# majidsina/rlmd

Measured on NVIDIA B200. Metric: investor-steps/sec (leverage sweep), higher is better.
Workload: dtype 2-bit codes, int32 counts, f64 log-wealth, f32 wealth

## Files before the change

include/rlmd_b200.h:

```cpp
#ifndef RLMD_B200_H
#define RLMD_B200_H

#include <stdint.h>

#ifdef __cplusplus
extern "C" {
#endif

#define B200_OK 0
#define B200_EINVAL (-1)
#define B200_ECUDA (-2)
#define B200_ELIMIT (-3)

#define B200_MAX_PEERS 8

const char* b200_last_error(void);
int b200_version(void);
int b200_device_info(int32_t* sm_count, int32_t* cc_major, int32_t* cc_minor);

enum {
  B200_LEV_DISCRETE = 0,
  B200_LEV_GBM = 1
};
enum {
  B200_SRC_STREAM = 0,
  B200_SRC_PHILOX = 1
};
enum {
  B200_MODE_CHAIN = 1,
  B200_MODE_LOG = 2
};

#define B200_MAX_GRID 64
#define B200_MAX_OUTCOMES 4

typedef struct b200_lev_desc {
  int64_t n_investors;
  int64_t ld_outcomes;
  int64_t investor_offset;
  int64_t ld_out;
  uint64_t seed;
  int32_t horizon;
  int32_t n_grid;
  int32_t n_outcomes;
  int32_t kind;
  int32_t source;
  int32_t mode;
  float value_0;
  float log_mean;
  float sigma;
  int32_t variant;
  uint32_t thresholds[B200_MAX_OUTCOMES];
  int32_t outcome_bits;
  int32_t flags;
} b200_lev_desc;

#define B200_LEV_FLAG_FINAL_ONLY 1
#define B200_LEV_FLAG_STATE_OUT 2
#define B200_LEV_FLAG_BESIDE_SWEEP 4

int b200_lev_sweep(const b200_lev_desc* desc, const void* outcomes,
                   const float* factors_host, float* data_T, double* log_w,
                   int32_t* counts, void* stream);

int b200_lev_chunk(const b200_lev_desc* desc, const void* outcomes,
                   const float* factors_host, int32_t t_begin, int32_t t_end,
                   void* state, float* dump, void* stream);

int b200_lev_draw(const b200_lev_desc* desc, void* out, void* stream);

int b200_lev_from_counts(const b200_lev_desc* desc, const int32_t* counts,
                         const float* factors_host, float* data_T, double* log_w,
                         void* stream);

int b200_lev_pack(const uint8_t* codes, int64_t n_investors, int32_t horizon,
                  int64_t ld_codes, uint8_t* packed, int64_t ld_packed, void* stream);
int b200_lev_pack_bits(const uint8_t* codes, int64_t n_investors, int32_t horizon,
                       int64_t ld_codes, uint8_t* packed, int64_t ld_packed, int32_t bits,
                       void* stream);

typedef struct b200_tally_plan {
  int64_t rows_cap;
  int64_t bins_cap;
  int32_t grid_cap;
  int32_t world;
} b200_tally_plan;

int64_t b200_tally_workspace_bytes(const b200_tally_plan* plan);
int64_t b200_tally_exchange_bytes(const b200_tally_plan* plan);

#define B200_TALLY_INFO_WORDS 8
int b200_tally_reset(const b200_tally_plan* plan, void* workspace, void* stream);

int b200_lev_tally(const b200_lev_desc* desc, const void* outcomes,
                   const b200_tally_plan* plan, void* workspace, int32_t* counts,
                   void* stream);

enum { B200_DT_U8 = 0, B200_DT_I32 = 1, B200_DT_I64 = 2, B200_DT_F32 = 3, B200_DT_F64 = 4 };
int b200_lev_ingest(const void* src, int32_t src_type, int64_t n_investors, int32_t horizon,
                    int64_t ld_src, int32_t n_outcomes, uint8_t* codes, int64_t ld_codes,
                    int32_t* counts, const b200_tally_plan* plan, void* workspace,
                    void* stream);

typedef struct b200_tally_peers {
  void* exchange[B200_MAX_PEERS];
  int32_t world, rank;
  uint32_t epoch;
  uint32_t reserved;
} b200_tally_peers;

int b200_tally_finalize(const b200_tally_plan* plan, void* workspace,
                        const b200_tally_peers* peers, int32_t phase, void* stream);

int b200_tally_stats(const b200_tally_plan* plan, void* workspace, const b200_lev_desc* desc,
                     const float* factors_host, int64_t n_total, int64_t top, double* stats,
                     void* stream);

int64_t b200_rowstats_workspace_bytes(int64_t rows);

int b200_rowstats(const float* values, int64_t rows, int64_t n, int64_t ld,
                  int64_t n_total, int64_t top, void* workspace, double* stats,
                  int32_t phase, void* stream);

int b200_rowstats_exchange(int32_t phase, int64_t out[5]);

enum { B200_ENV_COIN = 0, B200_ENV_DICE = 1, B200_ENV_GBM = 2, B200_ENV_DICE_SH = 3 };
enum { B200_INV_A = 0, B200_INV_B = 1, B200_INV_C = 2, B200_INV_INSURED = 3 };
#define B200_ENV_MAX_GAMBLES 8

typedef struct b200_env_desc {
  int32_t family;
  int32_t investor;
  int32_t n_gambles;
  int32_t stop_abs;
  double max_value, initial_value, min_value;
  double max_abs_action, min_reward, min_return;
  double max_return, min_weight, lev_factor;
  double returns[3];
  double probs[3];
  double sh_returns[3];
  double i_lev_factor, sh_lev_factor;
  double log_mean, vol;
  uint64_t seed;
} b200_env_desc;

int b200_menv_dims(const b200_env_desc* desc, int32_t* state_dim,
                   int32_t* action_dim, int32_t* risk_dim);

int b200_menv_reset(const b200_env_desc* desc, int64_t n_envs, double* wealth,
                    int32_t* time, double* state, const uint8_t* mask, void* stream);

int b200_menv_step(const b200_env_desc* desc, int64_t n_envs, double* wealth,
                   int32_t* time, const double* action, const double* returns_in,
                   uint64_t draw_index, double* next_state, double* reward,
                   uint8_t* done, double* risk, void* stream);

#define B200_REPLAY_MAX_STEPS 64

typedef struct b200_replay_desc {
  int64_t mem_size;
  int32_t state_dim;
  int32_t action_dim;
  float* state_memory;
  float* action_memory;
  float* reward_memory;
  float* next_state_memory;
  uint8_t* terminal_memory;
  int32_t* episode_start;
  int64_t* header;
} b200_replay_desc;

int b200_replay_reset(const b200_replay_desc* desc, void* stream);

int b200_replay_store(const b200_replay_desc* desc, const void* state, const void* action,
                      const void* reward, const void* next_state, const uint8_t* done,
                      int64_t count, int32_t is_f64, int64_t position, double reward_floor,
                      void* stream);

int b200_replay_store_host(const b200_replay_desc* desc, const double* state_host,
                           const double* action_host, double reward,
                           const double* next_state_host, int32_t done, int64_t position,
                           double reward_floor, void* stream);

int b200_replay_sample(const b200_replay_desc* desc, const int64_t* idx, int64_t n_batches,
                       int32_t batch, int64_t filled, int32_t multi_steps,
                       const float* gamma_pow_host, int32_t additive, uint64_t seed,
                       uint64_t draw_index, int64_t* out_idx, float* out_state,
                       float* out_action, float* out_reward, float* out_next_state,
                       uint8_t* out_done, int64_t* out_eff, void* stream);

int b200_replay_sample_counted(const b200_replay_desc* desc, int64_t n_batches, int32_t batch,
                               int32_t multi_steps, const float* gamma_pow_host, int32_t additive,
                               uint64_t seed, int64_t* counter, int64_t* out_idx, float* out_state,
                               float* out_action, float* out_reward, float* out_next_state,
                               uint8_t* out_done, int64_t* out_eff, void* stream);

typedef struct b200_collect_desc {
  b200_env_desc env;
  b200_replay_desc replay;
  int64_t n_envs;
  int64_t lane_len;
  double reward_floor;
} b200_collect_desc;

int b200_collect_reset(const b200_collect_desc* desc, double* wealth, int32_t* time,
                       double* cur_state, int64_t* counter, void* stream);

int b200_collect_step(const b200_collect_desc* desc, double* wealth, int32_t* time,
                      double* cur_state, const double* action, const double* returns_in,
                      int64_t* counter, double* reward, uint8_t* done, double* risk,
                      void* stream);

int b200_collect_sample(const b200_collect_desc* desc, const int64_t* idx, int64_t n_batches,
                        int32_t batch, int32_t multi_steps, const float* gamma_pow_host,
                        int32_t additive, uint64_t seed, int64_t* counter, int64_t* out_idx,
                        float* out_state, float* out_action, float* out_reward,
                        float* out_next_state, uint8_t* out_done, int64_t* out_eff,
                        void* stream);

int b200_menv_rollout(const b200_env_desc* desc, int64_t n_episodes, const double* action,
                      const double* returns_in, uint64_t draw_base, int32_t max_steps,
                      double* reward, int32_t* steps, double* risk, double* last_state,
                      void* stream);

#define B200_MARKET_MAX_ASSETS 128

typedef struct b200_market_desc {
  int32_t investor;
  int32_t n_assets;
  int32_t obs_days;
  int32_t time_length;
  double max_value, initial_value, min_value;
  double max_abs_action, min_reward, min_return;
  double max_return, min_weight, lev_factor;
} b200_market_desc;

int b200_market_dims(const b200_market_desc* desc, int32_t* state_dim, int32_t* action_dim,
                     int32_t* risk_dim);

int b200_market_reset(const b200_market_desc* desc, int64_t n_envs, double* wealth,
                      int32_t* time, const double* assets_in, double* assets, double* state,
                      const uint8_t* mask, void* stream);

int b200_market_step(const b200_market_desc* desc, int64_t n_envs, double* wealth,
                     int32_t* time, const double* assets, const double* action,
                     const double* next_assets, double* next_state, double* reward,
                     uint8_t* done, double* risk, void* stream);

#define B200_PEER_FLAG_ERROR_WORD (B200_MAX_PEERS * 8)
#define B200_PEER_FLAG_WORDS 128
typedef struct b200_peer_set {
  void* workspace[B200_MAX_PEERS];
  uint32_t* flags[B200_MAX_PEERS];
  void* stage[B200_MAX_PEERS];
  int64_t stage_rows;
  int32_t world, rank;
  uint32_t epoch;
  uint32_t reserved;
} b200_peer_set;
int64_t b200_rowstats_stage_bytes(int64_t rows, int32_t world);
int b200_rowstats_p2p(const float* values, int64_t rows, int64_t n, int64_t ld,
                      int64_t n_total, int64_t top, const b200_peer_set* peers,
                      double* stats, void* stream);

int b200_exchange_pack(const void* workspace, int64_t words_per_row, int64_t rows,
                       int64_t int_offset, int64_t int_count, int64_t dbl_offset,
                       int64_t dbl_count, double* staging, void* stream);
int b200_exchange_unpack(void* workspace, int64_t words_per_row, int64_t rows,
                         int64_t int_offset, int64_t int_count, int64_t dbl_offset,
                         int64_t dbl_count, const double* staging, void* stream);

int64_t b200_growth_workspace_bytes(int64_t rows);

int b200_gbm_valid(const double* state, const float* data_T, int64_t n, int64_t ld_T,
                   const float* lev_host, int32_t n_grid, double log_v0, double* out, void* stream);

int b200_gbm_growth_assemble(const double* base_row, const double* valid, const float* lev_host,
                             int32_t n_grid, int32_t horizon, int32_t n_q, const int32_t* pick_pos,
                             const int32_t* pick_neg, double* out, void* stream);
int b200_growth_exchange(int32_t phase, int64_t out[5]);
int b200_growth_summary(const double* log_w, const float* data_T, int64_t rows, int64_t n,
                        int64_t ld, int64_t ld_T, int64_t n_total, double log_v0,
                        int32_t horizon, const double* quantiles_host, int32_t n_q,
                        void* workspace, double* out, int32_t phase, void* stream);

enum { B200_BB_COIN = 0,
       B200_BB_DICE = 1   };
#define B200_BB_MAX_POINTS 128

typedef struct b200_bigbrain_desc {
  int64_t n_investors;
  int64_t ld_outcomes;
  int32_t horizon;
  int32_t n_points;
  int32_t kind;
  int32_t reserved;
  float value_0;
  float lev_factor32;
  double lev_factor64;
  double returns[3];
} b200_bigbrain_desc;

int b200_bigbrain_chunk(const b200_bigbrain_desc* desc, const uint8_t* outcomes,
                        const float* stop_vmin_host, const float* roll_host,
                        const double* lev0_host, int32_t s_begin, int32_t s_end, void* state,
                        float* dump, void* stream);

#ifdef __cplusplus
}
#endif
#endif
```

rlmd_b200/_lib.py:

```python
import ctypes as C
import os

_HERE = os.path.dirname(os.path.abspath(__file__))
LIB_PATH = os.path.join(_HERE, "librlmd_b200.so")

B200_OK, B200_EINVAL, B200_ECUDA, B200_ELIMIT = 0, -1, -2, -3
LEV_DISCRETE, LEV_GBM = 0, 1
SRC_STREAM, SRC_PHILOX = 0, 1
MODE_CHAIN, MODE_LOG = 1, 2
MAX_GRID, MAX_OUTCOMES = 64, 4


class LevDesc(C.Structure):
    _fields_ = [
        ("n_investors", C.c_int64),
        ("ld_outcomes", C.c_int64),
        ("investor_offset", C.c_int64),
        ("ld_out", C.c_int64),
        ("seed", C.c_uint64),
        ("horizon", C.c_int32),
        ("n_grid", C.c_int32),
        ("n_outcomes", C.c_int32),
        ("kind", C.c_int32),
        ("source", C.c_int32),
        ("mode", C.c_int32),
        ("value_0", C.c_float),
        ("log_mean", C.c_float),
        ("sigma", C.c_float),
        ("variant", C.c_int32),
        ("thresholds", C.c_uint32 * MAX_OUTCOMES),
        ("outcome_bits", C.c_int32),
        ("flags", C.c_int32),
    ]


LEV_FLAG_FINAL_ONLY, LEV_FLAG_STATE_OUT, LEV_FLAG_BESIDE_SWEEP = 1, 2, 4
MAX_PEERS = 8


class PeerSet(C.Structure):
    _fields_ = [
        ("workspace", C.c_void_p * MAX_PEERS),
        ("flags", C.c_void_p * MAX_PEERS),
        ("stage", C.c_void_p * MAX_PEERS),
        ("stage_rows", C.c_int64),
        ("world", C.c_int32),
        ("rank", C.c_int32),
        ("epoch", C.c_uint32),
        ("reserved", C.c_uint32),
    ]


class TallyPlan(C.Structure):
    _fields_ = [
        ("rows_cap", C.c_int64),
        ("bins_cap", C.c_int64),
        ("grid_cap", C.c_int32),
        ("world", C.c_int32),
    ]


class TallyPeers(C.Structure):
    _fields_ = [
        ("exchange", C.c_void_p * MAX_PEERS),
        ("world", C.c_int32),
        ("rank", C.c_int32),
        ("epoch", C.c_uint32),
        ("reserved", C.c_uint32),
    ]


DT_U8, DT_I32, DT_I64, DT_F32, DT_F64 = 0, 1, 2, 3, 4
TALLY_INFO_WORDS = 8
TALLY_MAX_HORIZON = (1 << 21) - 1

ENV_COIN, ENV_DICE, ENV_GBM, ENV_DICE_SH = 0, 1, 2, 3
INV_A, INV_B, INV_C, INV_INSURED = 0, 1, 2, 3
ENV_MAX_GAMBLES = 8


class EnvDesc(C.Structure):
    _fields_ = [
        ("family", C.c_int32),
        ("investor", C.c_int32),
        ("n_gambles", C.c_int32),
        ("stop_abs", C.c_int32),
        ("max_value", C.c_double),
        ("initial_value", C.c_double),
        ("min_value", C.c_double),
        ("max_abs_action", C.c_double),
        ("min_reward", C.c_double),
        ("min_return", C.c_double),
        ("max_return", C.c_double),
        ("min_weight", C.c_double),
        ("lev_factor", C.c_double),
        ("returns", C.c_double * 3),
        ("probs", C.c_double * 3),
        ("sh_returns", C.c_double * 3),
        ("i_lev_factor", C.c_double),
        ("sh_lev_factor", C.c_double),
        ("log_mean", C.c_double),
        ("vol", C.c_double),
        ("seed", C.c_uint64),
    ]


REPLAY_MAX_STEPS = 64


class ReplayDesc(C.Structure):
    _fields_ = [
        ("mem_size", C.c_int64),
        ("state_dim", C.c_int32),
        ("action_dim", C.c_int32),
        ("state_memory", C.c_void_p),
        ("action_memory", C.c_void_p),
        ("reward_memory", C.c_void_p),
        ("next_state_memory", C.c_void_p),
        ("terminal_memory", C.c_void_p),
        ("episode_start", C.c_void_p),
        ("header", C.c_void_p),
    ]


class MarketDesc(C.Structure):
    _fields_ = [
        ("investor", C.c_int32),
        ("n_assets", C.c_int32),
        ("obs_days", C.c_int32),
        ("time_length", C.c_int32),
        ("max_value", C.c_double),
        ("initial_value", C.c_double),
        ("min_value", C.c_double),
        ("max_abs_action", C.c_double),
        ("min_reward", C.c_double),
        ("min_return", C.c_double),
        ("max_return", C.c_double),
        ("min_weight", C.c_double),
        ("lev_factor", C.c_double),
    ]


MARKET_MAX_ASSETS = 128


class CollectDesc(C.Structure):
    _fields_ = [
        ("env", EnvDesc),
        ("replay", ReplayDesc),
        ("n_envs", C.c_int64),
        ("lane_len", C.c_int64),
        ("reward_floor", C.c_double),
    ]


BB_COIN, BB_DICE, BB_MAX_POINTS = 0, 1, 128


class BigBrainDesc(C.Structure):
    _fields_ = [
        ("n_investors", C.c_int64),
        ("ld_outcomes", C.c_int64),
        ("horizon", C.c_int32),
        ("n_points", C.c_int32),
        ("kind", C.c_int32),
        ("reserved", C.c_int32),
        ("value_0", C.c_float),
        ("lev_factor32", C.c_float),
        ("lev_factor64", C.c_double),
        ("returns", C.c_double * 3),
    ]


class B200Error(RuntimeError):
    def __init__(self, code, msg):
        super().__init__(f"rlmd_b200 error {code}: {msg}")
        self.code = code


if not os.path.isfile(LIB_PATH):
    raise ImportError(
        f"{LIB_PATH} is missing: build the CUDA library first (make, or __graft_entry__.build()); "
        "rlmd_b200 has no CPU fallback"
    )

lib = C.CDLL(LIB_PATH)

_vp, _i32, _i64 = C.c_void_p, C.c_int32, C.c_int64
_SIGNATURES = {
    "b200_last_error": (C.c_char_p, []),
    "b200_version": (C.c_int, []),
    "b200_device_info": (C.c_int, [C.POINTER(_i32)] * 3),
    "b200_lev_sweep": (C.c_int, [C.POINTER(LevDesc), _vp, C.POINTER(C.c_float), _vp, _vp, _vp, _vp]),
    "b200_lev_draw": (C.c_int, [C.POINTER(LevDesc), _vp, _vp]),
    "b200_lev_from_counts": (C.c_int, [C.POINTER(LevDesc), _vp, C.POINTER(C.c_float), _vp, _vp, _vp]),
    "b200_lev_pack": (C.c_int, [_vp, _i64, _i32, _i64, _vp, _i64, _vp]),
    "b200_lev_pack_bits": (C.c_int, [_vp, _i64, _i32, _i64, _vp, _i64, _i32, _vp]),
    "b200_lev_chunk": (C.c_int, [C.POINTER(LevDesc), _vp, C.POINTER(C.c_float), _i32, _i32, _vp, _vp, _vp]),
    "b200_menv_dims": (C.c_int, [C.POINTER(EnvDesc)] + [C.POINTER(_i32)] * 3),
    "b200_menv_reset": (C.c_int, [C.POINTER(EnvDesc), _i64, _vp, _vp, _vp, _vp, _vp]),
    "b200_menv_step": (C.c_int, [C.POINTER(EnvDesc), _i64, _vp, _vp, _vp, _vp, C.c_uint64, _vp, _vp, _vp, _vp, _vp]),
    "b200_replay_reset": (C.c_int, [C.POINTER(ReplayDesc), _vp]),
    "b200_replay_store": (C.c_int, [C.POINTER(ReplayDesc), _vp, _vp, _vp, _vp, _vp, _i64, _i32, _i64, C.c_double, _vp]),
    "b200_replay_store_host": (C.c_int, [C.POINTER(ReplayDesc), C.POINTER(C.c_double), C.POINTER(C.c_double),
                                         C.c_double, C.POINTER(C.c_double), _i32, _i64, C.c_double, _vp]),
    "b200_replay_sample": (C.c_int, [C.POINTER(ReplayDesc), _vp, _i64, _i32, _i64, _i32, C.POINTER(C.c_float), _i32,
                                     C.c_uint64, C.c_uint64, _vp, _vp, _vp, _vp, _vp, _vp, _vp, _vp]),
    "b200_replay_sample_counted": (C.c_int, [C.POINTER(ReplayDesc), _i64, _i32, _i32, C.POINTER(C.c_float), _i32,
                                             C.c_uint64, _vp, _vp, _vp, _vp, _vp, _vp, _vp, _vp, _vp]),
    "b200_exchange_pack": (C.c_int, [_vp, _i64, _i64, _i64, _i64, _i64, _i64, _vp, _vp]),
    "b200_exchange_unpack": (C.c_int, [_vp, _i64, _i64, _i64, _i64, _i64, _i64, _vp, _vp]),
    "b200_market_dims": (C.c_int, [C.POINTER(MarketDesc)] + [C.POINTER(_i32)] * 3),
    "b200_market_reset": (C.c_int, [C.POINTER(MarketDesc), _i64, _vp, _vp, _vp, _vp, _vp, _vp, _vp]),
    "b200_market_step": (C.c_int, [C.POINTER(MarketDesc), _i64, _vp, _vp, _vp, _vp, _vp, _vp, _vp, _vp, _vp, _vp]),
    "b200_collect_reset": (C.c_int, [C.POINTER(CollectDesc), _vp, _vp, _vp, _vp, _vp]),
    "b200_collect_step": (C.c_int, [C.POINTER(CollectDesc), _vp, _vp, _vp, _vp, _vp, _vp, _vp, _vp, _vp, _vp]),
    "b200_collect_sample": (C.c_int, [C.POINTER(CollectDesc), _vp, _i64, _i32, _i32, C.POINTER(C.c_float), _i32,
                                      C.c_uint64, _vp, _vp, _vp, _vp, _vp, _vp, _vp, _vp, _vp]),
    "b200_menv_rollout": (C.c_int, [C.POINTER(EnvDesc), _i64, _vp, _vp, C.c_uint64, _i32, _vp, _vp, _vp, _vp, _vp]),
    "b200_bigbrain_chunk": (C.c_int, [C.POINTER(BigBrainDesc), _vp, C.POINTER(C.c_float), C.POINTER(C.c_float),
                                      C.POINTER(C.c_double), _i32, _i32, _vp, _vp, _vp]),
    "b200_growth_workspace_bytes": (_i64, [_i64]),
    "b200_gbm_valid": (C.c_int, [_vp, _vp, _i64, _i64, C.POINTER(C.c_float), _i32, C.c_double, _vp, _vp]),
    "b200_gbm_growth_assemble": (C.c_int, [_vp, _vp, C.POINTER(C.c_float), _i32, _i32, _i32, _vp, _vp, _vp, _vp]),
    "b200_growth_exchange": (C.c_int, [_i32, C.POINTER(_i64)]),
    "b200_growth_summary": (C.c_int, [_vp, _vp, _i64, _i64, _i64, _i64, _i64, C.c_double, _i32, C.POINTER(C.c_double),
                                      _i32, _vp, _vp, _i32, _vp]),
    "b200_tally_workspace_bytes": (_i64, [C.POINTER(TallyPlan)]),
    "b200_tally_exchange_bytes": (_i64, [C.POINTER(TallyPlan)]),
    "b200_tally_reset": (C.c_int, [C.POINTER(TallyPlan), _vp, _vp]),
    "b200_lev_tally": (C.c_int, [C.POINTER(LevDesc), _vp, C.POINTER(TallyPlan), _vp, _vp, _vp]),
    "b200_lev_ingest": (C.c_int, [_vp, _i32, _i64, _i32, _i64, _i32, _vp, _i64, _vp, C.POINTER(TallyPlan), _vp, _vp]),
    "b200_tally_finalize": (C.c_int, [C.POINTER(TallyPlan), _vp, C.POINTER(TallyPeers), _i32, _vp]),
    "b200_tally_stats": (C.c_int, [C.POINTER(TallyPlan), _vp, C.POINTER(LevDesc), C.POINTER(C.c_float), _i64, _i64,
                                   _vp, _vp]),
    "b200_rowstats_workspace_bytes": (_i64, [_i64]),
    "b200_rowstats_stage_bytes": (_i64, [_i64, _i32]),
    "b200_rowstats": (C.c_int, [_vp, _i64, _i64, _i64, _i64, _i64, _vp, _vp, _i32, _vp]),
    "b200_rowstats_exchange": (C.c_int, [_i32, C.POINTER(_i64)]),
    "b200_rowstats_p2p": (C.c_int, [_vp, _i64, _i64, _i64, _i64, _i64, C.POINTER(PeerSet), _vp, _vp]),
}
EXPORTS = _SIGNATURES


def _bind():
    for name, (res, args) in _SIGNATURES.items():
        fn = getattr(lib, name)
        fn.restype = res
        fn.argtypes = args


_bind()


def check(rc: int) -> None:
    if rc != 0:
        raise B200Error(rc, lib.b200_last_error().decode("utf-8", "replace"))


def require_cuda():
    import torch

    if not torch.cuda.is_available():
        raise B200Error(B200_ECUDA, "no CUDA device: rlmd_b200 has no CPU fallback")


def stream_ptr():
    import torch

    raw = getattr(torch._C, "_cuda_getCurrentRawStream", None)
    if raw is not None:
        return C.c_void_p(raw(torch.cuda.current_device()))
    return C.c_void_p(torch.cuda.current_stream().cuda_stream)


def ptr(t):
    return C.c_void_p(0 if t is None else t.data_ptr())
```

rlmd_b200/csrc/tally.cu:

```cuda
#include <cooperative_groups.h>

#include <algorithm>
#include <cstdlib>
#include <cstring>

#include "tally.cuh"

namespace b200 {

struct BinEntry {
  unsigned long long key, count;
};
static_assert(sizeof(BinEntry) == 16, "one 16-byte vector per bin");

constexpr int MERGE_CHUNK = 2048;
constexpr int EX_FLAG_BYTES = 128;

struct LogTable {
  double lm[B200_MAX_OUTCOMES][B200_MAX_GRID];
};

struct TallyLayout {
  long long* header;
  unsigned long long* keysA; uint32_t* countsA; uint64_t capA;
  unsigned long long* ukeys; uint32_t* ucnt;
  float* wbuf; int64_t ldw;
  int64_t list_cap;
  BinEntry* concat; uint32_t* slot_of;
  unsigned long long* keysB; unsigned long long* countsB; uint32_t* posB; uint64_t capB;
  int32_t* blockcnt; int64_t nblk;
  int64_t bytes;
};

static uint64_t pow2_at_least(uint64_t v) {
  uint64_t p = 1;
  while (p < v) p <<= 1;
  return p;
}

static int plan_ok(const b200_tally_plan* p) {
  B200_REQUIRE(p != nullptr, "tally: plan is NULL");
  B200_REQUIRE(p->rows_cap >= 1 && p->rows_cap < ((int64_t)1 << 32), "tally: rows_cap must be in 1..2^32-1");
  B200_REQUIRE(p->bins_cap >= 1 && p->bins_cap < ((int64_t)1 << 31), "tally: bins_cap must be in 1..2^31-1");
  B200_REQUIRE(p->grid_cap >= 1 && p->grid_cap <= B200_MAX_GRID, "tally: grid_cap must be in 1..%d", B200_MAX_GRID);
  B200_REQUIRE(p->world >= 1 && p->world <= B200_MAX_PEERS, "tally: world must be in 1..%d", B200_MAX_PEERS);
  return 0;
}

static TallyLayout layout(const b200_tally_plan& p, void* base) {
  TallyLayout L;
  memset(&L, 0, sizeof(L));
  char* b = (char*)base;
  int64_t off = 0;
  auto take = [&](int64_t bytes) { char* r = b ? b + off : nullptr; off += (bytes + 255) & ~(int64_t)255; return r; };
  L.header = (long long*)take(TH_WORDS * 8);
  L.capA = pow2_at_least((uint64_t)std::max<int64_t>(2048, 2 * std::min(p.rows_cap, p.bins_cap)));
  L.list_cap = (int64_t)(L.capA / 2);
  L.keysA = (unsigned long long*)take((int64_t)L.capA * 8);
  L.countsA = (uint32_t*)take((int64_t)L.capA * 4);
  L.ukeys = (unsigned long long*)take(p.bins_cap * 8);
  L.ucnt = (uint32_t*)take(p.bins_cap * 4);
  L.ldw = (p.bins_cap + 3) & ~(int64_t)3;
  L.wbuf = (float*)take((int64_t)p.grid_cap * L.ldw * 4);
  if (p.world > 1) {
    const int64_t cat = (int64_t)p.world * L.list_cap;
    L.concat = (BinEntry*)take(cat * 16);
    L.slot_of = (uint32_t*)take(cat * 4);
    L.capB = pow2_at_least((uint64_t)std::max<int64_t>(1024, 2 * std::min(cat, p.bins_cap)));
    L.keysB = (unsigned long long*)take((int64_t)L.capB * 8);
    L.countsB = (unsigned long long*)take((int64_t)L.capB * 8);
    L.posB = (uint32_t*)take((int64_t)L.capB * 4);
    L.nblk = (cat + MERGE_CHUNK - 1) / MERGE_CHUNK;
    L.blockcnt = (int32_t*)take(L.nblk * 4);
  }
  L.bytes = off;
  return L;
}

static int64_t exchange_list_bytes(int64_t list_cap) { return 16 + list_cap * 16; }

int tally_device_view(const b200_tally_plan* plan, void* workspace, int32_t horizon, TallyDev* out) {
  if (int rc = plan_ok(plan)) return rc;
  B200_REQUIRE(workspace != nullptr, "tally: workspace is NULL");
  B200_REQUIRE(horizon <= TALLY_MAX_HORIZON, "tally: horizon must be < 2^%d (use b200_lev_sweep + b200_rowstats)",
               TALLY_COUNT_BITS);
  const TallyLayout L = layout(*plan, workspace);
  out->keys = L.keysA;
  out->counts = L.countsA;
  out->header = L.header;
  out->mask = L.capA - 1;
  return 0;
}

__global__ void __launch_bounds__(256)
tally_clear_kernel(unsigned long long* keys, uint32_t* counts32, unsigned long long* counts64, uint32_t* pos,
                   uint64_t cap) {
  for (uint64_t i = (uint64_t)blockIdx.x * blockDim.x + threadIdx.x; i < cap; i += (uint64_t)gridDim.x * blockDim.x) {
    keys[i] = TALLY_EMPTY;
    if (counts32) counts32[i] = 0;
    if (counts64) counts64[i] = 0;
    if (pos) pos[i] = 0xffffffffu;
  }
}

struct PeerView {
  BinEntry* list[B200_MAX_PEERS];
  long long* list_count[B200_MAX_PEERS];
  uint32_t* flags[B200_MAX_PEERS];
  int32_t world, rank;
  uint32_t epoch;
};

constexpr int COMPACT_PER = 8;
constexpr int COMPACT_CHUNK = 256 * COMPACT_PER;

template <bool MULTI>
__global__ void __launch_bounds__(256)
tally_compact_kernel(TallyDev t, unsigned long long* __restrict__ ukeys, uint32_t* __restrict__ ucnt,
                     int64_t out_cap, const __grid_constant__ PeerView P) {
  __shared__ BinEntry stage[COMPACT_CHUNK];
  __shared__ int n_s;
  __shared__ long long base_s;
  const uint64_t cap = t.mask + 1;
  const uint64_t base = (uint64_t)blockIdx.x * COMPACT_CHUNK;
  if (threadIdx.x == 0) n_s = 0;
  __syncthreads();
  unsigned long long key[COMPACT_PER];
  uint32_t cnt[COMPACT_PER];
#pragma unroll
  for (int u = 0; u < COMPACT_PER; ++u) {
    const uint64_t i = base + (uint64_t)u * 256 + threadIdx.x;
    key[u] = i < cap ? __ldcg(t.keys + i) : TALLY_EMPTY;
    cnt[u] = i < cap ? __ldcg(t.counts + i) : 0u;
  }
#pragma unroll
  for (int u = 0; u < COMPACT_PER; ++u) {
    if (key[u] == TALLY_EMPTY) continue;
    const uint64_t i = base + (uint64_t)u * 256 + threadIdx.x;
    t.keys[i] = TALLY_EMPTY;
    t.counts[i] = 0;
    const int p = atomicAdd(&n_s, 1);
    stage[p].key = key[u];
    stage[p].count = cnt[u];
  }
  __syncthreads();
  const int n = n_s;
  if (n > 0) {
    if (threadIdx.x == 0)
      base_s = (long long)atomicAdd(reinterpret_cast<unsigned long long*>(t.header + TH_LISTPOS), (unsigned long long)n);
    __syncthreads();
    BinEntry* list = MULTI ? P.list[P.rank] : nullptr;
    for (int j = threadIdx.x; j < n; j += 256) {
      const long long p = base_s + j;
      if (p < out_cap) {
        if (MULTI) list[p] = stage[j];
        else { ukeys[p] = stage[j].key; ucnt[p] = (uint32_t)stage[j].count; }
      } else {
        t.header[TH_OVERFLOW] = 1;
      }
    }
  }
  __shared__ int last_s;
  __threadfence();
  __syncthreads();
  if (threadIdx.x == 0) {
    const unsigned long long tk = atomicAdd(reinterpret_cast<unsigned long long*>(t.header + TH_TICKET), 1ull);
    last_s = tk == (unsigned long long)gridDim.x - 1;
  }
  __syncthreads();
  if (!last_s) return;
  __threadfence();
  if (threadIdx.x == 0) {
    const long long total = *reinterpret_cast<volatile long long*>(t.header + TH_LISTPOS);
    const long long m = total < out_cap ? total : out_cap;
    t.header[TH_LISTPOS] = 0;
    t.header[TH_TICKET] = 0;
    if (MULTI) *P.list_count[P.rank] = m;
    else t.header[TH_NBINS] = m;
  }
  if (MULTI) {
    __syncthreads();
    if (threadIdx.x < P.world && threadIdx.x != P.rank) {
      __threadfence_system();
      uint32_t* f = P.flags[threadIdx.x] + P.rank;
      asm volatile("st.release.sys.global.u32 [%0], %1;" ::"l"(f), "r"(P.epoch) : "memory");
    }
  }
}

__device__ __forceinline__ void ld_sys_entry(const BinEntry* p, unsigned long long& k, unsigned long long& c) {
  asm volatile("ld.relaxed.sys.global.v2.u64 {%0, %1}, [%2];" : "=l"(k), "=l"(c) : "l"(p));
}

__global__ void __launch_bounds__(256)
tally_merge_kernel(const __grid_constant__ PeerView P, long long* __restrict__ header, BinEntry* __restrict__ concat,
                   uint32_t* __restrict__ slot_of, unsigned long long* __restrict__ keysB,
                   unsigned long long* __restrict__ countsB, uint32_t* __restrict__ posB, uint64_t capB,
                   int64_t concat_cap) {
  __shared__ long long off_s[B200_MAX_PEERS + 1];
  __shared__ int ok_s;
  if (threadIdx.x == 0) ok_s = 1;
  __syncthreads();
  if (threadIdx.x < P.world && threadIdx.x != P.rank) {
    const uint32_t* f = P.flags[P.rank] + threadIdx.x;
    unsigned long long t0, t1;
    asm volatile("mov.u64 %0, %%globaltimer;" : "=l"(t0));
    for (;;) {
      uint32_t v;
      asm volatile("ld.acquire.sys.global.u32 %0, [%1];" : "=r"(v) : "l"(f) : "memory");
      if ((int32_t)(v - P.epoch) >= 0) break;
      __nanosleep(100);
      asm volatile("mov.u64 %0, %%globaltimer;" : "=l"(t1));
      if (t1 - t0 > 30000000000ull) { ok_s = 0; break; }
    }
  }
  __syncthreads();
  if (!ok_s) {
    if (threadIdx.x == 0) { header[TH_TIMEOUT] = 1; header[TH_CONCAT] = 0; }
    return;
  }
  if (threadIdx.x == 0) {
    long long acc = 0;
    for (int r = 0; r < P.world; ++r) {
      off_s[r] = acc;
      long long c;
      asm volatile("ld.relaxed.sys.global.s64 %0, [%1];" : "=l"(c) : "l"(P.list_count[r]));
      acc += c;
    }
    off_s[P.world] = acc;
  }
  __syncthreads();
  long long total = off_s[P.world];
  if (total > concat_cap) total = concat_cap;
  if (blockIdx.x == 0 && threadIdx.x == 0) header[TH_CONCAT] = total;
  uint64_t used = 1024;
  while (used < 2 * (uint64_t)total && used < capB) used <<= 1;
  const uint64_t mask = used - 1;
  for (long long p = (long long)blockIdx.x * blockDim.x + threadIdx.x; p < total;
       p += (long long)gridDim.x * blockDim.x) {
    int r = 0;
    while (r + 1 < P.world && p >= off_s[r + 1]) ++r;
    unsigned long long key, cnt;
    ld_sys_entry(P.list[r] + (p - off_s[r]), key, cnt);
    concat[p].key = key;
    concat[p].count = cnt;
    uint32_t found = 0xffffffffu;
    {
      uint64_t slot = tally_mix(key) & mask;
      for (int probe = 0; probe < TALLY_MAX_PROBE; ++probe) {
        unsigned long long cur = __ldcg(keysB + slot);
        if (cur == TALLY_EMPTY) {
          cur = atomicCAS(keysB + slot, TALLY_EMPTY, key);
          if (cur == TALLY_EMPTY) cur = key;
        }
        if (cur == key) {
          atomicAdd(countsB + slot, cnt);
          atomicMin(posB + slot, (uint32_t)p);
          found = (uint32_t)slot;
          break;
        }
        slot = (slot + 1) & mask;
      }
      if (found == 0xffffffffu) header[TH_OVERFLOW] = 1;
    }
    slot_of[p] = found;
  }
}

__global__ void __launch_bounds__(256)
tally_mark_kernel(const long long* __restrict__ header, const uint32_t* __restrict__ slot_of,
                  const uint32_t* __restrict__ posB, int32_t* __restrict__ blockcnt) {
  __shared__ long long red[32];
  const long long total = header[TH_CONCAT];
  const long long nchunks = (total + MERGE_CHUNK - 1) / MERGE_CHUNK;
  for (long long j = blockIdx.x; j < nchunks; j += gridDim.x) {
    const long long base = j * MERGE_CHUNK;
    long long c = 0;
    for (int u = 0; u < MERGE_CHUNK / 256; ++u) {
      const long long p = base + (long long)threadIdx.x * (MERGE_CHUNK / 256) + u;
      if (p < total) {
        const uint32_t s = slot_of[p];
        c += (s != 0xffffffffu && __ldcg(posB + s) == (uint32_t)p);
      }
    }
    c = block_sum(c, red);
    if (threadIdx.x == 0) blockcnt[j] = (int32_t)c;
    __syncthreads();
  }
}

__global__ void __launch_bounds__(256)
tally_unique_kernel(long long* __restrict__ header, const BinEntry* __restrict__ concat,
                    const uint32_t* __restrict__ slot_of, unsigned long long* __restrict__ keysB,
                    unsigned long long* __restrict__ countsB, uint32_t* __restrict__ posB,
                    const int32_t* __restrict__ blockcnt, unsigned long long* __restrict__ ukeys,
                    uint32_t* __restrict__ ucnt, int64_t bins_cap) {
  __shared__ long long red[32];
  __shared__ long long warp_tot[8];
  __shared__ long long base_s;
  const long long total = header[TH_CONCAT];
  const long long nchunks = (total + MERGE_CHUNK - 1) / MERGE_CHUNK;
  if (total == 0 && blockIdx.x == 0 && threadIdx.x == 0) header[TH_NBINS] = 0;
  for (long long j = blockIdx.x; j < nchunks; j += gridDim.x) {
    const long long base = j * MERGE_CHUNK;
    long long before = 0;
    for (long long i = threadIdx.x; i < j; i += 256) before += blockcnt[i];
    before = block_sum(before, red);
    if (threadIdx.x == 0) base_s = before;
    constexpr int PER = MERGE_CHUNK / 256;
    bool rep[PER];
    uint32_t slot[PER];
    int mine = 0;
#pragma unroll
    for (int u = 0; u < PER; ++u) {
      const long long p = base + (long long)threadIdx.x * PER + u;
      rep[u] = false;
      slot[u] = 0xffffffffu;
      if (p < total) {
        slot[u] = slot_of[p];
        rep[u] = slot[u] != 0xffffffffu && __ldcg(posB + slot[u]) == (uint32_t)p;
      }
      mine += rep[u];
    }
    const int lane = threadIdx.x & 31, wid = threadIdx.x >> 5;
    long long incl = mine;
#pragma unroll
    for (int o = 1; o < 32; o <<= 1) {
      const long long up = __shfl_up_sync(0xffffffffu, incl, o);
      if (lane >= o) incl += up;
    }
    if (lane == 31) warp_tot[wid] = incl;
    __syncthreads();
    long long pre = 0, blocktotal = 0;
#pragma unroll
    for (int w = 0; w < 8; ++w) {
      if (w < wid) pre += warp_tot[w];
      blocktotal += warp_tot[w];
    }
    long long outp = base_s + pre + incl - mine;
#pragma unroll
    for (int u = 0; u < PER; ++u) {
      if (!rep[u]) continue;
      const long long p = base + (long long)threadIdx.x * PER + u;
      if (outp < bins_cap) {
        ukeys[outp] = concat[p].key;
        ucnt[outp] = (uint32_t)__ldcg(countsB + slot[u]);
      } else {
        header[TH_OVERFLOW] = 1;
      }
      keysB[slot[u]] = TALLY_EMPTY;
      countsB[slot[u]] = 0;
      posB[slot[u]] = 0xffffffffu;
      ++outp;
    }
    if (base + MERGE_CHUNK >= total && threadIdx.x == 0) {
      const long long n = base_s + blocktotal;
      header[TH_NBINS] = n < bins_cap ? n : bins_cap;
    }
    __syncthreads();
  }
}

constexpr int SEL_THREADS = 1024;
constexpr int SL1 = 2048, SL2 = 2048, SL3 = 1024;
constexpr int SEL_MAX_CLUSTER = 16;

__device__ __forceinline__ void scan_hists(uint32_t* hist, int bins, int n_hist, uint32_t* warp_tot ) {
  const int grp = threadIdx.x >> 8, t = threadIdx.x & 255;
  const int lane = threadIdx.x & 31, wid = threadIdx.x >> 5;
  const int per = bins >> 8;
  uint32_t* h = hist + grp * bins + t * per;
  uint32_t local = 0;
  if (grp < n_hist)
    for (int i = 0; i < per; ++i) local += h[i];
  uint32_t incl = local;
#pragma unroll
  for (int o = 1; o < 32; o <<= 1) {
    const uint32_t up = __shfl_up_sync(0xffffffffu, incl, o);
    if (lane >= o) incl += up;
  }
  if (lane == 31) warp_tot[wid] = incl;
  __syncthreads();
  uint32_t pre = 0;
  for (int w = grp * 8; w < wid; ++w) pre += warp_tot[w];
  uint32_t run = pre + incl - local;
  if (grp < n_hist)
    for (int i = 0; i < per; ++i) { run += h[i]; h[i] = run; }
  __syncthreads();
}

__device__ __forceinline__ void find_rank(const uint32_t* pre, int bins, long long rank, int& bin, long long& rem) {
  int lo = 0, hi = bins - 1;
  while (lo < hi) {
    const int mid = (lo + hi) >> 1;
    if ((long long)pre[mid] > rank) hi = mid; else lo = mid + 1;
  }
  bin = lo;
  rem = rank - (lo > 0 ? (long long)pre[lo - 1] : 0);
}

__device__ __forceinline__ void push_hist(uint32_t* mine, uint32_t* leaders, int bins, int rank) {
  __syncthreads();
  if (rank != 0)
    for (int i = threadIdx.x; i < bins; i += blockDim.x) {
      const uint32_t v = mine[i];
      if (v != 0u) atomicAdd(leaders + i, v);
    }
}

struct SelShared {
  uint32_t hist[4 * SL2];
  double part_d[SEL_MAX_CLUSTER][6];
  long long part_i[SEL_MAX_CLUSTER][2];
  double res_d[4];
  long long res_i[16];
  uint32_t warp_tot[32];
  double red_d[32];
  double red_d2[32 * 6];
  long long red_i[32];
};

template <int N>
__device__ __forceinline__ void block_sum_n(double (&v)[N], double* scratch ) {
  const int lane = threadIdx.x & 31, wid = threadIdx.x >> 5;
#pragma unroll
  for (int q = 0; q < N; ++q) v[q] = warp_sum(v[q]);
  __syncthreads();
  if (lane == 0)
#pragma unroll
    for (int q = 0; q < N; ++q) scratch[q * 32 + wid] = v[q];
  __syncthreads();
  if (wid == 0) {
#pragma unroll
    for (int q = 0; q < N; ++q) {
      const double x = lane < (int)(blockDim.x >> 5) ? scratch[q * 32 + lane] : 0.0;
      v[q] = warp_sum(x);
    }
  }
}

template <int NK>
__global__ void __launch_bounds__(SEL_THREADS)
tally_select_kernel(long long* __restrict__ header, const unsigned long long* __restrict__ ukeys,
                    const uint32_t* __restrict__ ucnt, float* __restrict__ wbuf, int64_t ldw, int32_t H,
                    const __grid_constant__ LogTable lf, double logV0, int64_t n_total, int64_t top,
                    double* __restrict__ stats, int32_t SEL_CACHE ) {
  namespace cg = cooperative_groups;
  cg::cluster_group cluster = cg::this_cluster();
  const int C = (int)cluster.num_blocks(), r = (int)cluster.block_rank();
  __shared__ SelShared sh;
  extern __shared__ __align__(16) uint8_t dyn[];
  float* cw = reinterpret_cast<float*>(dyn);
  uint32_t* cc = reinterpret_cast<uint32_t*>(dyn) + SEL_CACHE;
  SelShared* L = cluster.map_shared_rank(&sh, 0);

  const int g = blockIdx.x / C;
  const long long B = header[TH_NBINS];
  const long long n = n_total, K = top;
  const double qnan = __longlong_as_double(0x7ff8000000000000LL);
  double* s = stats + (int64_t)g * 12;
  if (header[TH_TIMEOUT] != 0 || header[TH_OVERFLOW] != 0) {
    if (r == 0 && threadIdx.x < 12) s[threadIdx.x] = qnan;
    return;
  }
  const int tid = threadIdx.x, lane = threadIdx.x & 31;
#ifdef B200_TALLY_DEBUG
  int stamp_i = 0;
#define STAMP() do { if (r == 0 && tid == 0 && (g == 0 || g == (int)(gridDim.x / C) - 1)) { header[TH_DEBUG + (g == 0 ? 0 : 24) + stamp_i++] = clock64(); } } while (0)
#else
#define STAMP() do {} while (0)
#endif
  STAMP();
  const long long per = (((B + C - 1) / C) + 3) & ~3LL;
  const long long lo = min(B, (long long)r * per), hi = min(B, lo + per);
  const int m = (int)(hi - lo);
  float* __restrict__ w = wbuf + (int64_t)g * ldw + lo;
  const uint32_t* __restrict__ cnt = ucnt + lo;
  constexpr int REGS = 0;
  {
    double lm[NK];
#pragma unroll
    for (int k = 0; k < NK; ++k) lm[k] = lf.lm[k][g];
    for (int i = tid; i < m; i += SEL_THREADS) {
      int n1, n2, n3;
      tally_unkey(__ldg(ukeys + lo + i), n1, n2, n3);
      int nk[4];
      nk[1] = n1; nk[2] = NK >= 3 ? n2 : 0; nk[3] = NK >= 4 ? n3 : 0;
      nk[0] = H - nk[1] - nk[2] - nk[3];
      double lw = logV0;
#pragma unroll
      for (int k = 0; k < NK; ++k)
        if (nk[k] > 0) lw += (double)nk[k] * lm[k];
      const float x = (float)exp(lw);
      if (i < SEL_CACHE) { cw[i] = x; cc[i] = __ldg(cnt + i); }
      else w[i] = x;
    }
  }
  __syncthreads();
  auto far_w = [&](int i) { return i < REGS + SEL_CACHE ? cw[i - REGS] : w[i]; };
  auto far_c = [&](int i) { return i < REGS + SEL_CACHE ? cc[i - REGS] : cnt[i]; };
  auto sweep = [&](auto&& f) {
    for (int base = (tid & ~31); base < m; base += SEL_THREADS) {
      const int i = base + lane;
      const bool in = i < m;
      f(in ? far_w(i) : 0.f, in ? far_c(i) : 0u, in);
    }
  };

  for (int i = tid; i < SL1; i += SEL_THREADS) sh.hist[i] = 0;
  cluster.sync();
  STAMP();
  {
    double a0 = 0;
    long long c0 = 0;
    sweep([&](float x, uint32_t c, bool in) {
      a0 += (double)c * (double)x;
      c0 += c;
      warp_hist_add(sh.hist, float_key(x) >> 21, c, in);
    });
    STAMP();
    push_hist(sh.hist, L->hist, SL1, r);
    a0 = block_sum(a0, sh.red_d);
    c0 = block_sum(c0, sh.red_i);
    if (tid == 0) { L->part_d[r][0] = a0; L->part_i[r][0] = c0; }
  }
  cluster.sync();
  STAMP();
  if (r == 0) {
    if (tid == 0) {
      double sum_all = 0;
      long long cnt_all = 0;
      for (int q = 0; q < C; ++q) { sum_all += sh.part_d[q][0]; cnt_all += sh.part_i[q][0]; }
      if (cnt_all != n) header[TH_MISMATCH] = 1;
      const long long ninf = sh.hist[3], pinf = sh.hist[2044], nan = sh.hist[2047];
      const long long hi_ = pinf + nan;
      sh.res_i[0] = (hi_ + ninf) > 0; sh.res_i[1] = hi_ > 0 || ninf > n - K; sh.res_i[2] = hi_ > K || ninf > 0;
      sh.res_i[3] = nan > 0; sh.res_i[4] = nan > 0; sh.res_i[5] = nan > K;
      sh.res_d[0] = sum_all / (double)n;
    }
    scan_hists(sh.hist, SL1, 1, sh.warp_tot);
    if (tid < 4) {
      const long long ranks[4] = {(n - 1) / 2, n - K, n - K + (K - 1) / 2, (n - K - 1) / 2};
      int bin; long long rem;
      find_rank(sh.hist, SL1, ranks[tid], bin, rem);
      sh.res_i[8 + tid] = bin; sh.res_i[12 + tid] = rem;
    }
  }
  cluster.sync();
  uint32_t pre[4];
  long long rk[4];
#pragma unroll
  for (int j = 0; j < 4; ++j) { pre[j] = (uint32_t)L->res_i[8 + j]; rk[j] = L->res_i[12 + j]; }
  const double mean_a = L->res_d[0];
  STAMP();
  int rep[4];
  auto find_reps = [&]() {
#pragma unroll
    for (int j = 0; j < 4; ++j) {
      rep[j] = j;
#pragma unroll
      for (int q = 3; q >= 0; --q)
        if (q < j && pre[q] == pre[j]) rep[j] = q;
    }
  };
  auto copy_reps = [&](int bins) {
    for (int j = 1; j < 4; ++j)
      if (rep[j] != j)
        for (int i = tid; i < bins; i += SEL_THREADS) sh.hist[j * bins + i] = sh.hist[rep[j] * bins + i];
    __syncthreads();
  };
  find_reps();

  for (int j = 0; j < 4; ++j)
    if (rep[j] == j)
      for (int i = tid; i < SL2; i += SEL_THREADS) sh.hist[j * SL2 + i] = 0;
  cluster.sync();
  {
    sweep([&](float x, uint32_t c, bool in) {
      const uint32_t k = float_key(x);
      const uint32_t b1 = k >> 21, b2 = (k >> 10) & (SL2 - 1);
#pragma unroll
      for (int j = 0; j < 4; ++j)
        if (rep[j] == j) warp_hist_add(sh.hist + j * SL2, b2, c, in && b1 == pre[j]);
    });
    STAMP();
#pragma unroll
    for (int j = 0; j < 4; ++j)
      if (rep[j] == j) push_hist(sh.hist + j * SL2, L->hist + j * SL2, SL2, r);
  }
  STAMP();
  cluster.sync();
  STAMP();
  if (r == 0) {
    copy_reps(SL2);
    scan_hists(sh.hist, SL2, 4, sh.warp_tot);
    if (tid < 4) {
      int bin; long long rem;
      find_rank(sh.hist + tid * SL2, SL2, rk[tid], bin, rem);
      sh.res_i[8 + tid] = bin; sh.res_i[12 + tid] = rem;
    }
  }
  cluster.sync();
#pragma unroll
  for (int j = 0; j < 4; ++j) { pre[j] = (pre[j] << 11) | (uint32_t)L->res_i[8 + j]; rk[j] = L->res_i[12 + j]; }
  find_reps();
  STAMP();

  for (int j = 0; j < 4; ++j)
    if (rep[j] == j)
      for (int i = tid; i < SL3; i += SEL_THREADS) sh.hist[j * SL3 + i] = 0;
  cluster.sync();
  const uint32_t thr22 = pre[1];
  {
    double v[2] = {0, 0};
    long long c_gt = 0;
    sweep([&](float x, uint32_t c, bool in) {
      const uint32_t k = float_key(x);
      const uint32_t hi22 = k >> 10;
      const double cx = (double)c * (double)x;
      if (in && hi22 > thr22) { v[0] += cx; c_gt += c; }
      else if (in && hi22 < thr22) v[1] += cx;
#pragma unroll
      for (int j = 0; j < 4; ++j)
        if (rep[j] == j) warp_hist_add(sh.hist + j * SL3, k & (SL3 - 1), c, in && hi22 == pre[j]);
    });
    STAMP();
#pragma unroll
    for (int j = 0; j < 4; ++j)
      if (rep[j] == j) push_hist(sh.hist + j * SL3, L->hist + j * SL3, SL3, r);
    STAMP();
    block_sum_n<2>(v, sh.red_d2);
    c_gt = block_sum(c_gt, sh.red_i);
    if (tid == 0) { L->part_d[r][0] = v[0]; L->part_d[r][1] = v[1]; L->part_i[r][0] = c_gt; }
  }
  cluster.sync();
  if (r == 0) {
    copy_reps(SL3);
    scan_hists(sh.hist, SL3, 4, sh.warp_tot);
    if (tid < 4) {
      int bin; long long rem;
      find_rank(sh.hist + tid * SL3, SL3, rk[tid], bin, rem);
      sh.res_i[8 + tid] = bin; sh.res_i[12 + tid] = rem;
    }
    __syncthreads();
    const uint32_t thr_key = (pre[1] << 10) | (uint32_t)sh.res_i[8 + 1];
    const uint32_t thr_lo = thr_key & (SL3 - 1), base = thr_key & ~(uint32_t)(SL3 - 1);
    double f[5] = {0, 0, 0, 0, 0};
    const uint32_t* h3 = sh.hist + 1 * SL3;
    for (uint32_t b3 = tid; b3 < (uint32_t)SL3; b3 += SEL_THREADS) {
      const long long c = (long long)h3[b3] - (b3 > 0 ? (long long)h3[b3 - 1] : 0);
      f[4] += (double)c;
      if (c == 0 || b3 == thr_lo) continue;
      const double val = (double)c * (double)key_float(base | b3);
      if (b3 > thr_lo) { f[0] += val; f[2] += (double)c; } else { f[1] += val; f[3] += (double)c; }
    }
    block_sum_n<5>(f, sh.red_d2);
    if (tid == 0) {
      const long long fc_gt = (long long)f[2], fc_lt = (long long)f[3], fc_all = (long long)f[4];
      double coarse_gt = 0, coarse_lt = 0;
      long long cnt_gt = 0;
      for (int q = 0; q < C; ++q) { coarse_gt += sh.part_d[q][0]; coarse_lt += sh.part_d[q][1]; cnt_gt += sh.part_i[q][0]; }
      const double thr = (double)key_float(thr_key);
      const long long n_gt = cnt_gt + fc_gt, n_lt = (n - cnt_gt - fc_all) + fc_lt;
      const double sum_gt = fc_gt ? coarse_gt + f[0] : coarse_gt, sum_lt = fc_lt ? coarse_lt + f[1] : coarse_lt;
      const long long n_eq = n - n_gt - n_lt;
      const long long tt = K - n_gt;
      sh.res_i[6] = tt;
      sh.res_i[7] = n_eq - tt;
      sh.res_d[1] = (sum_gt + (tt > 0 ? (double)tt * thr : 0.0)) / (double)K;
      sh.res_d[2] = (sum_lt + (n_eq - tt > 0 ? (double)(n_eq - tt) * thr : 0.0)) / (double)(n - K);
    }
  }
  cluster.sync();
  uint32_t key_j[4];
#pragma unroll
  for (int j = 0; j < 4; ++j) key_j[j] = (pre[j] << 10) | (uint32_t)L->res_i[8 + j];
  const uint32_t thr_key = key_j[1];
  const double mean_t = L->res_d[1], mean_j = L->res_d[2];
  STAMP();

  double d[6] = {0, 0, 0, 0, 0, 0};
  sweep([&](float x, uint32_t ci, bool in) {
    const double c = (double)ci;
    const uint32_t k = float_key(x);
    const double xd = (double)x;
    const double da = xd - mean_a;
    d[4] += c * fabs(da);
    d[5] += c * (da * da);
    if (k < thr_key) { const double e = xd - mean_j; d[2] += c * fabs(e); d[3] += c * (e * e); }
    else if (k > thr_key) { const double e = xd - mean_t; d[0] += c * fabs(e); d[1] += c * (e * e); }
  });
  STAMP();
  block_sum_n<6>(d, sh.red_d2);
  STAMP();
  if (tid == 0) {
#pragma unroll
    for (int q = 0; q < 6; ++q) L->part_d[r][q] = d[q];
  }
  cluster.sync();
  STAMP();
  if (r == 0 && tid == 0) {
    double d0 = 0, d1 = 0, d2 = 0, d3 = 0, d4 = 0, d5 = 0;
    for (int q = 0; q < C; ++q) {
      d0 += sh.part_d[q][0]; d1 += sh.part_d[q][1]; d2 += sh.part_d[q][2];
      d3 += sh.part_d[q][3]; d4 += sh.part_d[q][4]; d5 += sh.part_d[q][5];
    }
    const double thr = (double)key_float(thr_key);
    const double dt = thr - mean_t, da = thr - mean_j;
    const double tt = (double)sh.res_i[6], ta = (double)sh.res_i[7];
    const double abs_top = d0 + (tt > 0 ? tt * fabs(dt) : 0.0);
    const double sq_top = d1 + (tt > 0 ? tt * dt * dt : 0.0);
    const double abs_adj = d2 + (ta > 0 ? ta * fabs(da) : 0.0);
    const double sq_adj = d3 + (ta > 0 ? ta * da * da : 0.0);
    s[0] = mean_a; s[1] = mean_t; s[2] = mean_j;
    s[3] = d4 / (double)n; s[4] = abs_top / (double)K; s[5] = abs_adj / (double)(n - K);
    s[6] = sqrt(d5 / (double)n); s[7] = sqrt(sq_top / (double)K); s[8] = sqrt(sq_adj / (double)(n - K));
    s[9] = (double)key_float(key_j[0]); s[10] = (double)key_float(key_j[2]); s[11] = (double)key_float(key_j[3]);
    const long long size[3] = {n, K, n - K};
    const double single[3] = {qnan, thr, (double)key_float(key_j[3])};
    for (int j = 0; j < 3; ++j) {
      if (sh.res_i[j]) { s[0 + j] = size[j] == 1 ? single[j] : qnan; s[3 + j] = qnan; s[6 + j] = qnan; }
      if (sh.res_i[3 + j]) s[9 + j] = qnan;
    }
  }
}

static void select_shape(int& cluster, int& cache) {
  static int c = [] {
    const char* e = getenv("B200_SELECT_CLUSTER");
    int x = e ? atoi(e) : 6;
    return x < 1 ? 1 : x > SEL_MAX_CLUSTER ? SEL_MAX_CLUSTER : x;
  }();
  static int k = [] {
    const char* e = getenv("B200_SELECT_CACHE");
    int x = e ? atoi(e) : 16384;
    return x < 0 ? 0 : x > 20480 ? 20480 : x;
  }();
  cluster = c;
  cache = k;
}

template <int K>
static int launch_select_k(int n_grid, long long* header, const unsigned long long* ukeys, const uint32_t* ucnt,
                           float* wbuf, int64_t ldw, int32_t H, const LogTable& lf, double logV0, int64_t n_total,
                           int64_t top, double* stats, bool beside_sweep, cudaStream_t st) {
  static bool attr_set[64] = {false};
  int dev = 0;
  B200_CUDA(cudaGetDevice(&dev));
  int C = 1, cache = 0;
  select_shape(C, cache);
  static const bool forced = getenv("B200_SELECT_CLUSTER") != nullptr;
  if (beside_sweep && !forced) C = 2;
  const size_t dyn = (size_t)cache * 8;
  if (dev < 64 && !attr_set[dev]) {
    B200_CUDA(cudaFuncSetAttribute(tally_select_kernel<K>, cudaFuncAttributeMaxDynamicSharedMemorySize, (int)dyn));
    if (C > 8) B200_CUDA(cudaFuncSetAttribute(tally_select_kernel<K>, cudaFuncAttributeNonPortableClusterSizeAllowed, 1));
    attr_set[dev] = true;
  }
  cudaLaunchConfig_t cfg;
  memset(&cfg, 0, sizeof(cfg));
  cfg.gridDim = dim3((unsigned)(n_grid * C));
  cfg.blockDim = dim3(SEL_THREADS);
  cfg.dynamicSmemBytes = dyn;
  cfg.stream = st;
  cudaLaunchAttribute at[1];
  at[0].id = cudaLaunchAttributeClusterDimension;
  at[0].val.clusterDim.x = (unsigned)C;
  at[0].val.clusterDim.y = 1;
  at[0].val.clusterDim.z = 1;
  cfg.attrs = at;
  cfg.numAttrs = 1;
  return check_cuda(cudaLaunchKernelEx(&cfg, tally_select_kernel<K>, header, ukeys, ucnt, wbuf, ldw, H, lf, logV0,
                                       n_total, top, stats, (int32_t)cache),
                    "tally_select launch");
}

static int grid_for(int64_t work, int threads, int per_sm) {
  const int64_t want = (work + threads - 1) / threads;
  const int64_t cap = (int64_t)sm_count() * per_sm;
  return (int)std::max<int64_t>(1, std::min(want, cap));
}

}

using namespace b200;

extern "C" int64_t b200_tally_workspace_bytes(const b200_tally_plan* plan) {
  if (plan_ok(plan)) return -1;
  return layout(*plan, nullptr).bytes;
}

extern "C" int64_t b200_tally_exchange_bytes(const b200_tally_plan* plan) {
  if (plan_ok(plan)) return -1;
  if (plan->world == 1) return 0;
  const TallyLayout L = layout(*plan, nullptr);
  return EX_FLAG_BYTES + 2 * ((exchange_list_bytes(L.list_cap) + 255) & ~(int64_t)255);
}

extern "C" int b200_tally_reset(const b200_tally_plan* plan, void* workspace, void* stream) {
  if (int rc = plan_ok(plan)) return rc;
  B200_REQUIRE(workspace != nullptr, "tally_reset: workspace is NULL");
  cudaStream_t st = (cudaStream_t)stream;
  const TallyLayout L = layout(*plan, workspace);
  B200_CUDA(cudaMemsetAsync(L.header, 0, TH_WORDS * 8, st));
  tally_clear_kernel<<<grid_for((int64_t)L.capA, 256, 8), 256, 0, st>>>(L.keysA, L.countsA, nullptr, nullptr, L.capA);
  if (plan->world > 1)
    tally_clear_kernel<<<grid_for((int64_t)L.capB, 256, 8), 256, 0, st>>>(L.keysB, nullptr, L.countsB, L.posB, L.capB);
  return check_cuda(cudaGetLastError(), "tally_reset launch");
}

extern "C" int b200_tally_finalize(const b200_tally_plan* plan, void* workspace, const b200_tally_peers* peers,
                                   int32_t phase, void* stream) {
  if (int rc = plan_ok(plan)) return rc;
  B200_REQUIRE(workspace != nullptr, "tally_finalize: workspace is NULL");
  B200_REQUIRE(phase >= -1 && phase <= 1, "tally_finalize: phase must be -1, 0 or 1");
  cudaStream_t st = (cudaStream_t)stream;
  const TallyLayout L = layout(*plan, workspace);
  TallyDev t{L.keysA, L.countsA, L.header, L.capA - 1};
  PeerView P;
  memset(&P, 0, sizeof(P));
  const int cgrid = (int)((L.capA + COMPACT_CHUNK - 1) / COMPACT_CHUNK);
  if (plan->world == 1) {
    if (phase == 1) return 0;
    tally_compact_kernel<false><<<cgrid, 256, 0, st>>>(t, L.ukeys, L.ucnt, std::min(plan->bins_cap, L.list_cap), P);
    return check_cuda(cudaGetLastError(), "tally_compact launch");
  }
  B200_REQUIRE(peers != nullptr, "tally_finalize: peers is NULL with world > 1");
  B200_REQUIRE(peers->world == plan->world && peers->rank >= 0 && peers->rank < peers->world,
               "tally_finalize: peers->world / rank do not fit the plan");
  B200_REQUIRE(peers->epoch >= 1, "tally_finalize: epoch starts at 1");
  const int64_t lbytes = (exchange_list_bytes(L.list_cap) + 255) & ~(int64_t)255;
  P.world = peers->world; P.rank = peers->rank; P.epoch = peers->epoch;
  for (int r = 0; r < peers->world; ++r) {
    B200_REQUIRE(peers->exchange[r] != nullptr, "tally_finalize: exchange buffer of rank %d is NULL", r);
    char* ex = (char*)peers->exchange[r];
    char* lst = ex + EX_FLAG_BYTES + (peers->epoch & 1) * lbytes;
    P.flags[r] = (uint32_t*)ex;
    P.list_count[r] = (long long*)lst;
    P.list[r] = (BinEntry*)(lst + 16);
  }
  if (phase != 1) {
    tally_compact_kernel<true><<<cgrid, 256, 0, st>>>(t, nullptr, nullptr, L.list_cap, P);
    B200_CUDA(cudaGetLastError());
  }
  if (phase == 0) return 0;
  const int64_t cat = (int64_t)plan->world * L.list_cap;
  tally_merge_kernel<<<sm_count() * 2, 256, 0, st>>>(P, L.header, L.concat, L.slot_of, L.keysB, L.countsB, L.posB,
                                                     L.capB, cat);
  B200_CUDA(cudaGetLastError());
  const unsigned mgrid = (unsigned)std::min<int64_t>(L.nblk, (int64_t)sm_count() * 2);
  tally_mark_kernel<<<mgrid, 256, 0, st>>>(L.header, L.slot_of, L.posB, L.blockcnt);
  B200_CUDA(cudaGetLastError());
  tally_unique_kernel<<<mgrid, 256, 0, st>>>(L.header, L.concat, L.slot_of, L.keysB, L.countsB, L.posB,
                                                        L.blockcnt, L.ukeys, L.ucnt, plan->bins_cap);
  return check_cuda(cudaGetLastError(), "tally_unique launch");
}

extern "C" int b200_tally_stats(const b200_tally_plan* plan, void* workspace, const b200_lev_desc* desc,
                                const float* factors_host, int64_t n_total, int64_t top, double* stats, void* stream) {
  if (int rc = plan_ok(plan)) return rc;
  B200_REQUIRE(workspace != nullptr && desc != nullptr && factors_host != nullptr && stats != nullptr,
               "tally_stats: NULL argument");
  B200_REQUIRE(desc->n_grid >= 1 && desc->n_grid <= plan->grid_cap, "tally_stats: n_grid must be in 1..grid_cap");
  B200_REQUIRE(desc->n_outcomes >= 2 && desc->n_outcomes <= B200_MAX_OUTCOMES, "tally_stats: n_outcomes out of range");
  B200_REQUIRE(desc->horizon >= 1 && desc->horizon <= TALLY_MAX_HORIZON, "tally_stats: horizon out of range");
  B200_REQUIRE(n_total >= 2 && n_total < ((int64_t)1 << 32), "tally_stats: need 2 <= n_total < 2^32");
  B200_REQUIRE(top >= 1 && top < n_total, "tally_stats: need 1 <= top < n_total (top=%lld)", (long long)top);
  cudaStream_t st = (cudaStream_t)stream;
  const TallyLayout L = layout(*plan, workspace);
  LogTable lf;
  for (int k = 0; k < B200_MAX_OUTCOMES; ++k)
    for (int g = 0; g < B200_MAX_GRID; ++g) {
      double v = 0.0;
      if (g < desc->n_grid && k < desc->n_outcomes) {
        const float m = factors_host[(int64_t)g * desc->n_outcomes + k];
        if (m < 0.0f) return set_error(B200_EINVAL, "tally_stats: factors must be >= 0 (m[%d][%d] = %g)", g, k, (double)m);
        v = log((double)m);
      }
      lf.lm[k][g] = v;
    }
  const double logV0 = log((double)desc->value_0);
  const bool beside = (desc->flags & B200_LEV_FLAG_BESIDE_SWEEP) != 0;
  switch (desc->n_outcomes) {
    case 2: return launch_select_k<2>(desc->n_grid, L.header, L.ukeys, L.ucnt, L.wbuf, L.ldw, desc->horizon, lf, logV0, n_total, top, stats, beside, st);
    case 3: return launch_select_k<3>(desc->n_grid, L.header, L.ukeys, L.ucnt, L.wbuf, L.ldw, desc->horizon, lf, logV0, n_total, top, stats, beside, st);
    default: return launch_select_k<4>(desc->n_grid, L.header, L.ukeys, L.ucnt, L.wbuf, L.ldw, desc->horizon, lf, logV0, n_total, top, stats, beside, st);
  }
}
```

rlmd_b200/csrc/tally.cuh:

```cuda
#pragma once
#include "common.cuh"

namespace b200 {

constexpr unsigned long long TALLY_EMPTY = ~0ull;
constexpr int TALLY_COUNT_BITS = 21;
constexpr int64_t TALLY_MAX_HORIZON = (1 << TALLY_COUNT_BITS) - 1;

enum {
  TH_NBINS = 0,
  TH_OVERFLOW = 1,
  TH_BAD = 2,
  TH_TIMEOUT = 3,
  TH_MISMATCH = 4,
  TH_TICKET = 9,
  TH_LISTPOS = 10,
  TH_CONCAT = 11,
  TH_DEBUG = 16,
  TH_WORDS = 64
};

struct TallyDev {
  unsigned long long* keys;
  uint32_t* counts;
  long long* header;
  uint64_t mask;
};

__host__ __device__ __forceinline__ uint64_t tally_mix(uint64_t x) {
  x ^= x >> 33; x *= 0xff51afd7ed558ccdull;
  x ^= x >> 33; x *= 0xc4ceb9fe1a85ec53ull;
  x ^= x >> 33;
  return x;
}

__host__ __device__ __forceinline__ uint64_t tally_key(int n1, int n2, int n3) {
  return (uint64_t)(uint32_t)n1 | ((uint64_t)(uint32_t)n2 << TALLY_COUNT_BITS) |
         ((uint64_t)(uint32_t)n3 << (2 * TALLY_COUNT_BITS));
}
__host__ __device__ __forceinline__ void tally_unkey(uint64_t key, int& n1, int& n2, int& n3) {
  n1 = (int)(key & TALLY_MAX_HORIZON);
  n2 = (int)((key >> TALLY_COUNT_BITS) & TALLY_MAX_HORIZON);
  n3 = (int)((key >> (2 * TALLY_COUNT_BITS)) & TALLY_MAX_HORIZON);
}

constexpr int TALLY_MAX_PROBE = 256;
__device__ __forceinline__ void tally_insert(const TallyDev& t, uint64_t key, uint32_t add) {
  uint64_t slot = tally_mix(key) & t.mask;
  for (int probe = 0; probe < TALLY_MAX_PROBE; ++probe) {
    unsigned long long cur = __ldcg(t.keys + slot);
    if (cur == TALLY_EMPTY) {
      cur = atomicCAS(t.keys + slot, TALLY_EMPTY, (unsigned long long)key);
      if (cur == TALLY_EMPTY) cur = key;
    }
    if (cur == key) { atomicAdd(t.counts + slot, add); return; }
    slot = (slot + 1) & t.mask;
  }
  t.header[TH_OVERFLOW] = 1;
}

int tally_device_view(const ::b200_tally_plan* plan, void* workspace, int32_t horizon, TallyDev* out);

}
```

rlmd_b200/tally.py:

```python
from __future__ import annotations

import ctypes as C
from typing import Optional

import numpy as np
import torch

from . import _lib
from ._lib import LevDesc, TallyPeers, TallyPlan, check, lib, ptr, require_cuda, stream_ptr

_SRC_TYPES = {
    torch.uint8: _lib.DT_U8, torch.bool: _lib.DT_U8, torch.int32: _lib.DT_I32, torch.int64: _lib.DT_I64,
    torch.float32: _lib.DT_F32, torch.float64: _lib.DT_F64,
}

DEFAULT_BINS_CAP = 1 << 22


class TallyOverflow(RuntimeError):
    """More distinct count tuples than the plan's bins_cap: use lev_sweep + rowstats for this input."""


class TallyUnavailable(TallyOverflow):
    """The ranks of the group cannot map each other's memory (no peer access): the tally's exchange cannot be
    set up; callers take the general path (lev_sweep + rowstats with the NCCL exchange), like on overflow."""


class TallyExchange:

    def __init__(self, nbytes: int, group, device):
        import torch.distributed as dist
        import torch.distributed._symmetric_memory as symm

        self.world, self.rank = dist.get_world_size(group), dist.get_rank(group)
        self.buf = symm.empty((nbytes + 7) // 8, dtype=torch.int64, device=device)
        self.buf.zero_()
        self.handle = symm.rendezvous(self.buf, group)
        self.ptrs = [int(p) for p in self.handle.buffer_ptrs]
        torch.cuda.synchronize(device)
        dist.barrier(group=group)
        self.epoch = 0

    def next_peers(self) -> TallyPeers:
        self.epoch += 1
        p = TallyPeers()
        p.world, p.rank, p.epoch = self.world, self.rank, self.epoch
        for r in range(self.world):
            p.exchange[r] = self.ptrs[r]
        return p


class FinalTally:

    def __init__(self, rows_cap: int, *, device="cuda", group=None, bins_cap: Optional[int] = None,
                 grid_cap: int = _lib.MAX_GRID, world_rows: Optional[int] = None):
        require_cuda()
        self.dev = torch.device(device)
        if self.dev.index is None:
            self.dev = torch.device("cuda", torch.cuda.current_device())
        self.group = group
        world = 1
        if group is not None:
            import torch.distributed as dist

            world = dist.get_world_size(group)
        rows_cap = max(int(rows_cap), 1)
        total = int(world_rows) if world_rows is not None else rows_cap * world
        self.plan = TallyPlan()
        self.plan.rows_cap = rows_cap
        self.plan.bins_cap = int(bins_cap) if bins_cap is not None else max(1024, min(total, DEFAULT_BINS_CAP))
        self.plan.grid_cap = int(grid_cap)
        self.plan.world = world
        nbytes = lib.b200_tally_workspace_bytes(C.byref(self.plan))
        if nbytes < 0:
            raise _lib.B200Error(_lib.B200_EINVAL, lib.b200_last_error().decode())
        with torch.cuda.device(self.dev):
            self.ws = torch.empty((nbytes // 8,), dtype=torch.int64, device=self.dev)
            self.exchange = None
            if world > 1:
                self.exchange = TallyExchange(lib.b200_tally_exchange_bytes(C.byref(self.plan)), group, self.dev)
            check(lib.b200_tally_reset(C.byref(self.plan), ptr(self.ws), stream_ptr()))
        self._staging = None
        self.rows = 0
        self.horizon = None

    def reset(self) -> None:
        with torch.cuda.device(self.dev):
            check(lib.b200_tally_reset(C.byref(self.plan), ptr(self.ws), stream_ptr()))
        self.rows = 0

    def _note(self, n: int, h: int) -> None:
        if self.horizon is not None and self.rows > 0 and self.horizon != h:
            raise ValueError("every row block of one sweep must have the same horizon")
        if self.rows + n > self.plan.rows_cap:
            raise ValueError(f"more than rows_cap = {self.plan.rows_cap} rows in one sweep")
        if h > _lib.TALLY_MAX_HORIZON:
            raise ValueError("the tally path needs horizon < 2^21")
        self.horizon = h
        self.rows += n

    def add(self, outcomes, n_outcomes: int, *, counts: Optional[torch.Tensor] = None,
            codes_out: Optional[torch.Tensor] = None) -> None:
        from .engine import PackedCodes

        k = int(n_outcomes)
        with torch.cuda.device(self.dev):
            if isinstance(outcomes, PackedCodes) or (outcomes.dtype == torch.uint8 and codes_out is None):
                packed = isinstance(outcomes, PackedCodes)
                data = outcomes.data if packed else outcomes
                n, h = outcomes.shape
                if not data.is_cuda or data.dim() != 2 or (n > 1 and data.stride(1) != 1):
                    raise ValueError("outcomes must be a [N,H] CUDA tensor with unit inner stride")
                self._note(n, h)
                d = LevDesc()
                d.kind, d.mode, d.source = _lib.LEV_DISCRETE, _lib.MODE_LOG, _lib.SRC_STREAM
                d.n_investors, d.horizon, d.n_grid, d.n_outcomes = n, h, 1, k
                d.value_0 = 1.0
                d.outcome_bits = outcomes.bits if packed else 8
                d.ld_outcomes = data.stride(0) if n > 1 else data.shape[1]
                check(lib.b200_lev_tally(C.byref(d), ptr(data), C.byref(self.plan), ptr(self.ws), ptr(counts),
                                         stream_ptr()))
                return
            t = outcomes
            if t.dtype not in _SRC_TYPES:
                raise TypeError(f"outcomes of dtype {t.dtype} are not an accepted format")
            if not t.is_cuda or t.dim() != 2 or (t.shape[0] > 1 and t.stride(1) != 1):
                raise ValueError("outcomes must be a [N,H] CUDA tensor with unit inner stride")
            n, h = t.shape
            self._note(n, h)
            ld = t.stride(0) if n > 1 else max(t.stride(0), h)
            ldc = 0
            if codes_out is not None:
                if codes_out.dtype != torch.uint8 or codes_out.shape[0] != n or codes_out.shape[1] < h:
                    raise ValueError("codes_out must be uint8 [N, >=H]")
                ldc = codes_out.stride(0) if n > 1 else codes_out.shape[1]
            check(lib.b200_lev_ingest(ptr(t), _SRC_TYPES[t.dtype], n, h, ld, k, ptr(codes_out), ldc, ptr(counts),
                                      C.byref(self.plan), ptr(self.ws), stream_ptr()))

    def add_host(self, host: torch.Tensor, n_outcomes: int, *, chunk_bytes: int = 256 << 20,
                 horizon: Optional[int] = None) -> int:
        from .engine import PackedCodes, _copy_stream

        packed = isinstance(host, PackedCodes)
        src = host.data if packed else host
        if src.is_cuda or src.dim() != 2:
            raise ValueError("add_host takes a 2-D host tensor (or PackedCodes over one)")
        n = src.shape[0]
        h = host.horizon if packed else src.shape[1]
        if n == 0:
            return 0
        if src.stride(1) != 1:
            src = src.contiguous()
        if src.dtype == torch.bool:
            src = src.view(torch.uint8)
        width = src.shape[1]
        row_bytes = width * src.element_size()
        rows = int(max(1, min(n, chunk_bytes // max(row_bytes, 1))))
        with torch.cuda.device(self.dev):
            key = (src.dtype, rows, width)
            if self._staging is None or self._staging[0] != key:
                self._staging = (key, [torch.empty((rows, width), dtype=src.dtype, device=self.dev) for _ in range(2)],
                                 [torch.cuda.Event() for _ in range(2)], [torch.cuda.Event() for _ in range(2)])
            _, bufs, ready, done = self._staging
            comp = torch.cuda.current_stream()
            copy = _copy_stream(self.dev)
            copy.wait_stream(comp)
            for i, r0 in enumerate(range(0, n, rows)):
                m = min(rows, n - r0)
                b = bufs[i & 1]
                if i >= 2:
                    copy.wait_event(done[i & 1])
                with torch.cuda.stream(copy):
                    b[:m].copy_(src[r0:r0 + m], non_blocking=True)
                    ready[i & 1].record(copy)
                comp.wait_event(ready[i & 1])
                self.add(PackedCodes(b[:m], h, host.bits) if packed else b[:m], n_outcomes)
                done[i & 1].record(comp)
            copy.wait_event(done[0])
            copy.wait_event(done[1])
        return n * row_bytes

    def finalize(self) -> None:
        with torch.cuda.device(self.dev):
            peers = self.exchange.next_peers() if self.exchange is not None else None
            check(lib.b200_tally_finalize(C.byref(self.plan), ptr(self.ws), C.byref(peers) if peers else None, -1,
                                          stream_ptr()))
        self.rows = 0

    def stats(self, factors: np.ndarray, value_0: float, horizon: int, *, n_total: int, top: int,
              beside_sweep: bool = False) -> torch.Tensor:
        f = np.ascontiguousarray(factors, dtype=np.float32)
        if f.ndim != 2:
            raise ValueError("factors must be [G,K]")
        g, k = f.shape
        out = torch.empty((g, 12), dtype=torch.float64, device=self.dev)
        d = LevDesc()
        d.kind, d.mode, d.source = _lib.LEV_DISCRETE, _lib.MODE_LOG, _lib.SRC_STREAM
        d.horizon, d.n_outcomes, d.value_0 = int(horizon), k, float(value_0)
        d.flags = _lib.LEV_FLAG_BESIDE_SWEEP if beside_sweep else 0
        with torch.cuda.device(self.dev):
            for g0 in range(0, g, self.plan.grid_cap):
                tile = np.ascontiguousarray(f[g0:g0 + self.plan.grid_cap])
                d.n_grid = tile.shape[0]
                check(lib.b200_tally_stats(C.byref(self.plan), ptr(self.ws), C.byref(d),
                                           tile.ctypes.data_as(C.POINTER(C.c_float)), int(n_total), int(top),
                                           ptr(out[g0:]), stream_ptr()))
        return out

    def info(self) -> dict:
        w = self.ws[:_lib.TALLY_INFO_WORDS]
        if self.group is not None:
            import torch.distributed as dist

            w = w.clone()
            dist.all_reduce(w, op=dist.ReduceOp.MAX, group=self.group)
        w = w.cpu().tolist()
        return {"bins": w[0], "overflow": bool(w[1]), "bad_outcomes": w[2], "timed_out": bool(w[3]),
                "count_mismatch": bool(w[4])}

    def check(self) -> dict:
        i = self.info()
        if i["overflow"] or i["bad_outcomes"] or i["timed_out"] or i["count_mismatch"]:
            self.reset()
        if i["timed_out"]:
            raise RuntimeError("rlmd_b200: a rank's bins did not arrive within 30 s (peer-memory exchange)")
        if i["bad_outcomes"]:
            raise ValueError(f"{i['bad_outcomes']} outcomes outside 0..K-1: the reference would use such a value as "
                             "the factor itself (lev/lev_exp.py:541); not supported")
        if i["overflow"]:
            raise TallyOverflow(f"more than {self.plan.bins_cap} distinct outcome-count tuples")
        if i["count_mismatch"]:
            raise RuntimeError("rlmd_b200: the tallied rows do not add up to n_total")
        return i
```

Before: 21420 billion.

## Select top-k by log-wealth lattice histogram with radix fallback

The compact and merge kernels now track a bounding box of outcome counts per tally. The select kernel uses it to bin entries directly by log-wealth over a known range, so it can locate quantile ranks with one histogram plus a small per-bin candidate set instead of multi-level float-key radix passes. It falls back to the radix path when the box is degenerate, K>3, a bin holds too many candidates, or a flag forces radix. This adds shared-memory candidate buffers, an extra 2-byte bin cache per entry, and more complex correctness conditions.

```diff
diff --git a/include/rlmd_b200.h b/include/rlmd_b200.h
--- a/include/rlmd_b200.h
+++ b/include/rlmd_b200.h
@@ -58,6 +58,7 @@
 #define B200_LEV_FLAG_FINAL_ONLY 1
 #define B200_LEV_FLAG_STATE_OUT 2
 #define B200_LEV_FLAG_BESIDE_SWEEP 4
+#define B200_LEV_FLAG_RADIX_SELECT 8
 
 int b200_lev_sweep(const b200_lev_desc* desc, const void* outcomes,
                    const float* factors_host, float* data_T, double* log_w,
diff --git a/oracle/tally_lwsel_oracle.py b/oracle/tally_lwsel_oracle.py
--- /dev/null
+++ b/oracle/tally_lwsel_oracle.py
@@ -0,0 +1,85 @@
+import math
+
+import numpy as np
+
+NBINS = 2048
+CAND = 512
+KEY_ZERO, KEY_INF = 0x80000000, 0xFF800000
+
+
+def float_key(w: np.ndarray) -> np.ndarray:
+    b = np.ascontiguousarray(w, dtype=np.float32).view(np.uint32).astype(np.uint64)
+    k = np.where(b & 0x80000000, ~b & 0xFFFFFFFF, b | 0x80000000)
+    k = np.where((b & 0x7FFFFFFF) > 0x7F800000, 0xFFFFFFFF, k)
+    return k.astype(np.uint64)
+
+
+def log_wealth(tuples: np.ndarray, lm: np.ndarray, value_0: float) -> np.ndarray:
+    lw = np.full(tuples.shape[0], math.log(float(np.float32(value_0))))
+    for k in range(tuples.shape[1]):
+        nk = tuples[:, k].astype(np.float64)
+        with np.errstate(invalid="ignore"):
+            lw = lw + np.where(nk > 0, nk * lm[k], 0.0)
+    return lw
+
+
+def lw_range(tuples: np.ndarray, lm: np.ndarray, value_0: float):
+    k = tuples.shape[1]
+    if k > 3 or len(tuples) == 0 or not np.isfinite(lm).all():
+        return None
+    h = float(tuples[0].sum())
+    a = (int(tuples[:, 1].min()), int(tuples[:, 1].max()))
+    b = (int(tuples[:, 2].min()), int(tuples[:, 2].max())) if k == 3 else (0, 0)
+    logv0 = math.log(float(np.float32(value_0)))
+    vals = []
+    for n2 in b:
+        for n1 in a:
+            v = logv0 + (h - n1 - n2) * lm[0] + n1 * lm[1]
+            if k == 3:
+                v += n2 * lm[2]
+            vals.append(v)
+    lo, hi = min(vals), max(vals)
+    return (lo, hi) if hi > lo and math.isfinite(hi - lo) else None
+
+
+def select(lw: np.ndarray, wealth: np.ndarray, counts: np.ndarray, rng, top: int, cand: int = CAND):
+    n, k = int(counts.sum()), int(top)
+    lo, hi = rng
+    t = (lw - lo) * (NBINS / (hi - lo))
+    b = np.where(t >= NBINS - 1, NBINS - 1, np.where(t > 0, np.floor(np.where(t > 0, t, 0)), 0)).astype(np.int64)
+    pre = np.cumsum(np.bincount(b, weights=counts, minlength=NBINS).astype(np.int64))
+    keys = float_key(wealth)
+    out = []
+    for j, rk in enumerate(((n - 1) // 2, n - k, n - k + (k - 1) // 2, (n - k - 1) // 2)):
+        bq = int(np.searchsorted(pre, rk, side="right"))
+        rem = rk - (int(pre[bq - 1]) if bq > 0 else 0)
+        inb, below, above = b == bq, b < bq, b > bq
+        if int(inb.sum()) > cand:
+            return None
+        ck, cc = keys[inb], counts[inb]
+        order = np.lexsort((cc, ck))
+        ck, cc = ck[order], cc[order]
+        v = int(ck[np.searchsorted(np.cumsum(cc), rem, side="right")])
+        lo_max = int(keys[below].max()) if below.any() else 0
+        hi_min = int(keys[above].min()) if above.any() else 0xFFFFFFFF
+        apart = v in (KEY_ZERO, KEY_INF) or lo_max < v < hi_min
+        if not lo_max <= v <= hi_min or (j == 1 and not apart):
+            return None
+        out.append(v)
+        if j == 1:
+            b1 = bq
+    thr, above = out[1], b > b1
+    sat = (keys == KEY_INF) | (keys == KEY_ZERO)
+    n_gt = int(counts[above & ~sat].sum()) + int(counts[(b == b1) & (keys > thr)].sum())
+    for key in (KEY_INF, KEY_ZERO):
+        if thr != key:
+            n_gt += int(counts[above & (keys == key)].sum())
+    vals = np.array(out, dtype=np.uint64)
+    return key_float(vals), n_gt
+
+
+def key_float(k: np.ndarray) -> np.ndarray:
+    k = np.asarray(k, dtype=np.uint64)
+    b = np.where(k & 0x80000000, k & 0x7FFFFFFF, ~k & 0xFFFFFFFF)
+    b = np.where(k == 0xFFFFFFFF, 0x7FC00000, b)
+    return b.astype(np.uint32).view(np.float32)
diff --git a/rlmd_b200/_lib.py b/rlmd_b200/_lib.py
--- a/rlmd_b200/_lib.py
+++ b/rlmd_b200/_lib.py
@@ -34,7 +34,7 @@
     ]
 
 
-LEV_FLAG_FINAL_ONLY, LEV_FLAG_STATE_OUT, LEV_FLAG_BESIDE_SWEEP = 1, 2, 4
+LEV_FLAG_FINAL_ONLY, LEV_FLAG_STATE_OUT, LEV_FLAG_BESIDE_SWEEP, LEV_FLAG_RADIX_SELECT = 1, 2, 4, 8
 MAX_PEERS = 8
 
 
diff --git a/rlmd_b200/csrc/tally.cu b/rlmd_b200/csrc/tally.cu
--- a/rlmd_b200/csrc/tally.cu
+++ b/rlmd_b200/csrc/tally.cu
@@ -111,6 +111,25 @@
   uint32_t epoch;
 };
 
+__device__ __forceinline__ void box_add(uint32_t (&b)[4], unsigned long long key) {
+  int n1, n2, n3;
+  tally_unkey(key, n1, n2, n3);
+  b[0] = max(b[0], (uint32_t)(TALLY_MAX_HORIZON - n1)); b[1] = max(b[1], (uint32_t)n1);
+  b[2] = max(b[2], (uint32_t)(TALLY_MAX_HORIZON - n2)); b[3] = max(b[3], (uint32_t)n2);
+}
+__device__ __forceinline__ void box_flush(const uint32_t (&b)[4], long long* dst, uint32_t* s ) {
+  if (threadIdx.x < 4) s[threadIdx.x] = 0;
+  __syncthreads();
+#pragma unroll
+  for (int q = 0; q < 4; ++q) {
+    const uint32_t m = __reduce_max_sync(0xffffffffu, b[q]);
+    if ((threadIdx.x & 31) == 0 && m != 0u) atomicMax(s + q, m);
+  }
+  __syncthreads();
+  if (threadIdx.x < 4 && s[threadIdx.x] != 0u)
+    atomicMax(reinterpret_cast<unsigned long long*>(dst) + threadIdx.x, (unsigned long long)s[threadIdx.x]);
+}
+
 constexpr int COMPACT_PER = 8;
 constexpr int COMPACT_CHUNK = 256 * COMPACT_PER;
 
@@ -121,6 +140,8 @@
   __shared__ BinEntry stage[COMPACT_CHUNK];
   __shared__ int n_s;
   __shared__ long long base_s;
+  __shared__ uint32_t box_s[4];
+  uint32_t box[4] = {0, 0, 0, 0};
   const uint64_t cap = t.mask + 1;
   const uint64_t base = (uint64_t)blockIdx.x * COMPACT_CHUNK;
   if (threadIdx.x == 0) n_s = 0;
@@ -139,12 +160,14 @@
     const uint64_t i = base + (uint64_t)u * 256 + threadIdx.x;
     t.keys[i] = TALLY_EMPTY;
     t.counts[i] = 0;
+    if (!MULTI) box_add(box, key[u]);
     const int p = atomicAdd(&n_s, 1);
     stage[p].key = key[u];
     stage[p].count = cnt[u];
   }
   __syncthreads();
   const int n = n_s;
+  if (!MULTI && n > 0) box_flush(box, t.header + TH_BOX_ACC, box_s);
   if (n > 0) {
     if (threadIdx.x == 0)
       base_s = (long long)atomicAdd(reinterpret_cast<unsigned long long*>(t.header + TH_LISTPOS), (unsigned long long)n);
@@ -176,7 +199,14 @@
     t.header[TH_LISTPOS] = 0;
     t.header[TH_TICKET] = 0;
     if (MULTI) *P.list_count[P.rank] = m;
-    else t.header[TH_NBINS] = m;
+    else {
+      t.header[TH_NBINS] = m;
+      t.header[TH_RADIX] = 0;
+      for (int q = 0; q < 4; ++q) {
+        t.header[TH_BOX + q] = *reinterpret_cast<volatile long long*>(t.header + TH_BOX_ACC + q);
+        t.header[TH_BOX_ACC + q] = 0;
+      }
+    }
   }
   if (MULTI) {
     __syncthreads();
@@ -232,7 +262,11 @@
   __syncthreads();
   long long total = off_s[P.world];
   if (total > concat_cap) total = concat_cap;
-  if (blockIdx.x == 0 && threadIdx.x == 0) header[TH_CONCAT] = total;
+  if (blockIdx.x == 0 && threadIdx.x == 0) {
+    header[TH_CONCAT] = total;
+    header[TH_RADIX] = 0;
+    for (int q = 0; q < 4; ++q) header[TH_BOX + q] = 0;
+  }
   uint64_t used = 1024;
   while (used < 2 * (uint64_t)total && used < capB) used <<= 1;
   const uint64_t mask = used - 1;
@@ -298,6 +332,8 @@
   __shared__ long long red[32];
   __shared__ long long warp_tot[8];
   __shared__ long long base_s;
+  __shared__ uint32_t box_s[4];
+  uint32_t box[4] = {0, 0, 0, 0};
   const long long total = header[TH_CONCAT];
   const long long nchunks = (total + MERGE_CHUNK - 1) / MERGE_CHUNK;
   if (total == 0 && blockIdx.x == 0 && threadIdx.x == 0) header[TH_NBINS] = 0;
@@ -343,6 +379,7 @@
       if (!rep[u]) continue;
       const long long p = base + (long long)threadIdx.x * PER + u;
       if (outp < bins_cap) {
+        box_add(box, concat[p].key);
         ukeys[outp] = concat[p].key;
         ucnt[outp] = (uint32_t)__ldcg(countsB + slot[u]);
       } else {
@@ -359,6 +396,7 @@
     }
     __syncthreads();
   }
+  box_flush(box, header + TH_BOX, box_s);
 }
 
 constexpr int SEL_THREADS = 1024;
@@ -408,15 +446,24 @@
     }
 }
 
+constexpr int CAND = 512;
+constexpr int CAND_CTA = 256;
+
 struct SelShared {
   uint32_t hist[4 * SL2];
+  uint32_t ext[4][2];
+  uint32_t ext_cta[4][2];
+  uint32_t cand_cta[2][4][CAND_CTA];
+  int ncand_cta[4], base_cta[4];
+  uint32_t sel[4];
+  int ncand[4], found[4], lat_ok;
   double part_d[SEL_MAX_CLUSTER][6];
-  long long part_i[SEL_MAX_CLUSTER][2];
+  long long part_i[SEL_MAX_CLUSTER][5];
   double res_d[4];
   long long res_i[16];
   uint32_t warp_tot[32];
   double red_d[32];
-  double red_d2[32 * 6];
+  double red_d2[32 * 7];
   long long red_i[32];
 };
 
@@ -444,7 +491,8 @@
 tally_select_kernel(long long* __restrict__ header, const unsigned long long* __restrict__ ukeys,
                     const uint32_t* __restrict__ ucnt, float* __restrict__ wbuf, int64_t ldw, int32_t H,
                     const __grid_constant__ LogTable lf, double logV0, int64_t n_total, int64_t top,
-                    double* __restrict__ stats, int32_t SEL_CACHE ) {
+                    double* __restrict__ stats, int32_t SEL_CACHE ,
+                    int32_t force_radix) {
   namespace cg = cooperative_groups;
   cg::cluster_group cluster = cg::this_cluster();
   const int C = (int)cluster.num_blocks(), r = (int)cluster.block_rank();
@@ -452,6 +500,7 @@
   extern __shared__ __align__(16) uint8_t dyn[];
   float* cw = reinterpret_cast<float*>(dyn);
   uint32_t* cc = reinterpret_cast<uint32_t*>(dyn) + SEL_CACHE;
+  uint16_t* cb = reinterpret_cast<uint16_t*>(cc + SEL_CACHE);
   SelShared* L = cluster.map_shared_rank(&sh, 0);
 
   const int g = blockIdx.x / C;
@@ -477,28 +526,70 @@
   float* __restrict__ w = wbuf + (int64_t)g * ldw + lo;
   const uint32_t* __restrict__ cnt = ucnt + lo;
   constexpr int REGS = 0;
-  {
-    double lm[NK];
-#pragma unroll
-    for (int k = 0; k < NK; ++k) lm[k] = lf.lm[k][g];
-    for (int i = tid; i < m; i += SEL_THREADS) {
-      int n1, n2, n3;
-      tally_unkey(__ldg(ukeys + lo + i), n1, n2, n3);
-      int nk[4];
-      nk[1] = n1; nk[2] = NK >= 3 ? n2 : 0; nk[3] = NK >= 4 ? n3 : 0;
-      nk[0] = H - nk[1] - nk[2] - nk[3];
-      double lw = logV0;
-#pragma unroll
-      for (int k = 0; k < NK; ++k)
-        if (nk[k] > 0) lw += (double)nk[k] * lm[k];
-      const float x = (float)exp(lw);
-      if (i < SEL_CACHE) { cw[i] = x; cc[i] = __ldg(cnt + i); }
-      else w[i] = x;
+  double lm[NK];
+#pragma unroll
+  for (int k = 0; k < NK; ++k) lm[k] = lf.lm[k][g];
+  auto lw_of = [&](unsigned long long key) {
+    int n1, n2, n3;
+    tally_unkey(key, n1, n2, n3);
+    int nk[4];
+    nk[1] = n1; nk[2] = NK >= 3 ? n2 : 0; nk[3] = NK >= 4 ? n3 : 0;
+    nk[0] = H - nk[1] - nk[2] - nk[3];
+    double lw = logV0;
+#pragma unroll
+    for (int k = 0; k < NK; ++k)
+      if (nk[k] > 0) lw += (double)nk[k] * lm[k];
+    return lw;
+  };
+  bool lat = false;
+  double lw_lo = 0.0, lw_scale = 0.0;
+  if (NK <= 3 && !force_radix) {
+    const long long M = TALLY_MAX_HORIZON;
+    const long long a[2] = {M - header[TH_BOX + 0], header[TH_BOX + 1]}, b[2] = {M - header[TH_BOX + 2], header[TH_BOX + 3]};
+    bool fin = a[0] <= a[1] && b[0] <= b[1];
+#pragma unroll
+    for (int k = 0; k < NK; ++k) fin = fin && isfinite(lm[k]);
+    if (fin) {
+      double lo_ = INFINITY, hi_ = -INFINITY;
+      for (int u = 0; u < 4; ++u) {
+        const double n1 = (double)a[u & 1], n2 = NK >= 3 ? (double)b[u >> 1] : 0.0;
+        double v = logV0 + ((double)H - n1 - n2) * lm[0] + n1 * lm[1];
+        if (NK >= 3) v += n2 * lm[NK >= 3 ? 2 : 0];
+        lo_ = fmin(lo_, v);
+        hi_ = fmax(hi_, v);
+      }
+      if (hi_ > lo_ && isfinite(hi_ - lo_)) { lat = true; lw_lo = lo_; lw_scale = (double)SL1 / (hi_ - lo_); }
+    }
+  }
+  auto lw_bin = [&](double lw) -> uint32_t {
+    const double t = (lw - lw_lo) * lw_scale;
+    return t >= (double)(SL1 - 1) ? (uint32_t)(SL1 - 1) : t > 0.0 ? (uint32_t)t : 0u;
+  };
+  if (lat) {
+    for (int i = tid; i < SL1; i += SEL_THREADS) sh.hist[i] = 0;
+    cluster.sync();
+  }
+  double a0 = 0;
+  long long c0 = 0, pinf = 0;
+  for (int i = tid; i < m; i += SEL_THREADS) {
+    const double lw = lw_of(__ldg(ukeys + lo + i));
+    const float x = (float)exp(lw);
+    const uint32_t c = __ldg(cnt + i);
+    if (i < SEL_CACHE) { cw[i] = x; cc[i] = c; }
+    else w[i] = x;
+    if (lat) {
+      const uint32_t bn = lw_bin(lw);
+      if (i < SEL_CACHE) cb[i] = (uint16_t)bn;
+      atomicAdd(sh.hist + bn, c);
+      a0 += (double)c * (double)x;
+      c0 += c;
+      if (isinf(x)) pinf += c;
     }
   }
   __syncthreads();
   auto far_w = [&](int i) { return i < REGS + SEL_CACHE ? cw[i - REGS] : w[i]; };
   auto far_c = [&](int i) { return i < REGS + SEL_CACHE ? cc[i - REGS] : cnt[i]; };
+  auto far_b = [&](int i) { return i < SEL_CACHE ? (uint32_t)cb[i] : lw_bin(lw_of(__ldg(ukeys + lo + i))); };
   auto sweep = [&](auto&& f) {
     for (int base = (tid & ~31); base < m; base += SEL_THREADS) {
       const int i = base + lane;
@@ -506,178 +597,374 @@
       f(in ? far_w(i) : 0.f, in ? far_c(i) : 0u, in);
     }
   };
-
-  for (int i = tid; i < SL1; i += SEL_THREADS) sh.hist[i] = 0;
-  cluster.sync();
-  STAMP();
-  {
-    double a0 = 0;
-    long long c0 = 0;
-    sweep([&](float x, uint32_t c, bool in) {
-      a0 += (double)c * (double)x;
-      c0 += c;
-      warp_hist_add(sh.hist, float_key(x) >> 21, c, in);
-    });
+  const long long ranks[4] = {(n - 1) / 2, n - K, n - K + (K - 1) / 2, (n - K - 1) / 2};
+  uint32_t key_j[4];
+  bool radix = !lat;
+
+  if (lat) {
     STAMP();
     push_hist(sh.hist, L->hist, SL1, r);
-    a0 = block_sum(a0, sh.red_d);
-    c0 = block_sum(c0, sh.red_i);
-    if (tid == 0) { L->part_d[r][0] = a0; L->part_i[r][0] = c0; }
-  }
-  cluster.sync();
-  STAMP();
-  if (r == 0) {
-    if (tid == 0) {
-      double sum_all = 0;
-      long long cnt_all = 0;
-      for (int q = 0; q < C; ++q) { sum_all += sh.part_d[q][0]; cnt_all += sh.part_i[q][0]; }
-      if (cnt_all != n) header[TH_MISMATCH] = 1;
-      const long long ninf = sh.hist[3], pinf = sh.hist[2044], nan = sh.hist[2047];
-      const long long hi_ = pinf + nan;
-      sh.res_i[0] = (hi_ + ninf) > 0; sh.res_i[1] = hi_ > 0 || ninf > n - K; sh.res_i[2] = hi_ > K || ninf > 0;
-      sh.res_i[3] = nan > 0; sh.res_i[4] = nan > 0; sh.res_i[5] = nan > K;
-      sh.res_d[0] = sum_all / (double)n;
-    }
-    scan_hists(sh.hist, SL1, 1, sh.warp_tot);
-    if (tid < 4) {
-      const long long ranks[4] = {(n - 1) / 2, n - K, n - K + (K - 1) / 2, (n - K - 1) / 2};
-      int bin; long long rem;
-      find_rank(sh.hist, SL1, ranks[tid], bin, rem);
-      sh.res_i[8 + tid] = bin; sh.res_i[12 + tid] = rem;
-    }
-  }
-  cluster.sync();
-  uint32_t pre[4];
-  long long rk[4];
-#pragma unroll
-  for (int j = 0; j < 4; ++j) { pre[j] = (uint32_t)L->res_i[8 + j]; rk[j] = L->res_i[12 + j]; }
-  const double mean_a = L->res_d[0];
-  STAMP();
-  int rep[4];
-  auto find_reps = [&]() {
+    {
+      double v[3] = {a0, (double)c0, (double)pinf};
+      block_sum_n<3>(v, sh.red_d2);
+      if (tid == 0) { L->part_d[r][0] = v[0]; L->part_i[r][0] = (long long)v[1]; L->part_i[r][1] = (long long)v[2]; }
+    }
+    if (tid < 4) { sh.ext_cta[tid][0] = 0u; sh.ext_cta[tid][1] = 0xffffffffu; sh.ncand_cta[tid] = 0; }
+    cluster.sync();
+    STAMP();
+    if (r == 0) {
+      if (tid == 0) {
+        double sum_all = 0;
+        long long cnt_all = 0, inf_all = 0;
+        for (int q = 0; q < C; ++q) { sum_all += sh.part_d[q][0]; cnt_all += sh.part_i[q][0]; inf_all += sh.part_i[q][1]; }
+        if (cnt_all != n) header[TH_MISMATCH] = 1;
+        sh.res_i[0] = inf_all > 0; sh.res_i[1] = inf_all > 0; sh.res_i[2] = inf_all > K;
+        sh.res_i[3] = 0; sh.res_i[4] = 0; sh.res_i[5] = 0;
+        sh.res_d[0] = sum_all / (double)n;
+      }
+      if (tid < 4) { sh.ncand[tid] = 0; sh.found[tid] = 0; sh.ext[tid][0] = 0u; sh.ext[tid][1] = 0xffffffffu; }
+      scan_hists(sh.hist, SL1, 1, sh.warp_tot);
+      if (tid < 4) {
+        int bin; long long rem;
+        find_rank(sh.hist, SL1, ranks[tid], bin, rem);
+        sh.res_i[8 + tid] = bin; sh.res_i[12 + tid] = rem;
+      }
+    }
+    cluster.sync();
+    STAMP();
+    int bq[4], rep[4];
 #pragma unroll
     for (int j = 0; j < 4; ++j) {
+      bq[j] = (int)L->res_i[8 + j];
       rep[j] = j;
 #pragma unroll
       for (int q = 3; q >= 0; --q)
-        if (q < j && pre[q] == pre[j]) rep[j] = q;
-    }
-  };
-  auto copy_reps = [&](int bins) {
-    for (int j = 1; j < 4; ++j)
-      if (rep[j] != j)
-        for (int i = tid; i < bins; i += SEL_THREADS) sh.hist[j * bins + i] = sh.hist[rep[j] * bins + i];
-    __syncthreads();
-  };
-  find_reps();
-
-  for (int j = 0; j < 4; ++j)
-    if (rep[j] == j)
-      for (int i = tid; i < SL2; i += SEL_THREADS) sh.hist[j * SL2 + i] = 0;
-  cluster.sync();
-  {
-    sweep([&](float x, uint32_t c, bool in) {
-      const uint32_t k = float_key(x);
-      const uint32_t b1 = k >> 21, b2 = (k >> 10) & (SL2 - 1);
+        if (q < j && bq[q] == bq[j]) rep[j] = q;
+    }
+    {
+      double v[7] = {0, 0, 0, 0, 0, 0, 0};
+      uint32_t ext_lo[4] = {0u, 0u, 0u, 0u}, ext_hi[4] = {~0u, ~0u, ~0u, ~0u};
+      for (int i = tid; i < m; i += SEL_THREADS) {
+        const int bn = (int)far_b(i);
+        const float x = far_w(i);
+        const uint32_t c = far_c(i), k = float_key(x);
+        if (bn > bq[1]) {
+          if (isinf(x)) v[3] += (double)c;
+          else if (x == 0.f) v[4] += (double)c;
+          else { v[0] += (double)c * (double)x; v[2] += (double)c; }
+        } else if (bn < bq[1]) {
+          if (isinf(x)) v[5] += (double)c;
+          else if (x == 0.f) v[6] += (double)c;
+          else v[1] += (double)c * (double)x;
+        }
+#pragma unroll
+        for (int j = 0; j < 4; ++j) {
+          if (bn < bq[j]) ext_lo[j] = max(ext_lo[j], k);
+          else if (bn > bq[j]) ext_hi[j] = min(ext_hi[j], k);
+          else if (rep[j] == j) {
+            const int p = atomicAdd(&sh.ncand_cta[j], 1);
+            if (p < CAND_CTA) { sh.cand_cta[0][j][p] = k; sh.cand_cta[1][j][p] = c; }
+          }
+        }
+      }
+#pragma unroll
+      for (int j = 0; j < 4; ++j) {
+        const uint32_t a = __reduce_max_sync(0xffffffffu, ext_lo[j]), b = __reduce_min_sync(0xffffffffu, ext_hi[j]);
+        if (lane == 0) { atomicMax(&sh.ext_cta[j][0], a); atomicMin(&sh.ext_cta[j][1], b); }
+      }
+      STAMP();
+      block_sum_n<7>(v, sh.red_d2);
+      if (tid == 0) {
+        L->part_d[r][0] = v[0]; L->part_d[r][1] = v[1];
+#pragma unroll
+        for (int q = 0; q < 5; ++q) L->part_i[r][q] = (long long)v[2 + q];
+      }
+      if (tid < 8) {
+        const int j = tid >> 1;
+        if (tid & 1) atomicMin(&L->ext[j][1], sh.ext_cta[j][1]);
+        else atomicMax(&L->ext[j][0], sh.ext_cta[j][0]);
+      }
+      if (tid < 4 && rep[tid] == tid)
+        sh.base_cta[tid] = atomicAdd(&L->ncand[tid], sh.ncand_cta[tid] <= CAND_CTA ? sh.ncand_cta[tid] : CAND + 1);
+      __syncthreads();
+#pragma unroll
+      for (int j = 0; j < 4; ++j) {
+        if (rep[j] != j) continue;
+        const int nl = min(sh.ncand_cta[j], CAND_CTA), b0 = sh.base_cta[j];
+        for (int p = tid; p < nl && b0 + p < CAND; p += SEL_THREADS) {
+          L->hist[j * CAND + b0 + p] = sh.cand_cta[0][j][p];
+          L->hist[4 * CAND + j * CAND + b0 + p] = sh.cand_cta[1][j][p];
+        }
+      }
+    }
+    cluster.sync();
+    STAMP();
+    if (r == 0) {
+      int mq[4], off[5];
+      off[0] = 0;
+#pragma unroll
+      for (int j = 0; j < 4; ++j) { mq[j] = rep[j] == j ? min(sh.ncand[j], CAND) : 0; off[j + 1] = off[j] + mq[j]; }
+      const int gi = tid >> 3, sub = tid & 7;
+      for (int c0 = 0; c0 < off[4]; c0 += SEL_THREADS / 8) {
+        const int idx = c0 + gi;
+        const bool in = idx < off[4];
+        int j = 0, oj = 0, mj = mq[0], pos = 0;
+#pragma unroll
+        for (int q = 1; q < 4; ++q)
+          if (idx >= off[q]) { j = q; oj = off[q]; mj = mq[q]; }
+        const int t = idx - oj;
+        uint32_t kt = 0, ct = 0;
+        long long below = 0, eq = 0;
+        if (in) {
+          const uint32_t* ck = sh.hist + j * CAND;
+          const uint32_t* ccn = sh.hist + 4 * CAND + j * CAND;
+          kt = ck[t]; ct = ccn[t];
+          for (int u = sub; u < mj; u += 8) {
+            const uint32_t ku = ck[u], cu = ccn[u];
+            if (ku < kt) below += cu;
+            else if (ku == kt) eq += cu;
+            pos += ku < kt || (ku == kt && (cu < ct || (cu == ct && u < t)));
+          }
+        }
+#pragma unroll
+        for (int o = 4; o > 0; o >>= 1) {
+          below += __shfl_xor_sync(0xffffffffu, below, o);
+          eq += __shfl_xor_sync(0xffffffffu, eq, o);
+          pos += __shfl_xor_sync(0xffffffffu, pos, o);
+        }
+        if (in && sub == 0) {
+          sh.hist[8 * CAND + j * CAND + pos] = kt;
+          sh.hist[12 * CAND + j * CAND + pos] = ct;
+#pragma unroll
+          for (int q = 0; q < 4; ++q) {
+            const long long rem = sh.res_i[12 + q];
+            if (rep[q] == j && below <= rem && rem < below + eq) { sh.sel[q] = kt; sh.found[q] = 1; }
+          }
+        }
+      }
+      __syncthreads();
+      const uint32_t thr_key = sh.sel[1];
+      const int m1 = rep[1] == 0 ? mq[0] : mq[1];
+      double f[5] = {0, 0, 0, 0, 0};
+      for (int t = tid; t < m1; t += SEL_THREADS) {
+        const uint32_t k = sh.hist[8 * CAND + rep[1] * CAND + t];
+        const long long c = sh.hist[12 * CAND + rep[1] * CAND + t];
+        f[4] += (double)c;
+        if (k == thr_key) continue;
+        const double val = (double)c * (double)key_float(k);
+        if (k > thr_key) { f[0] += val; f[2] += (double)c; } else { f[1] += val; f[3] += (double)c; }
+      }
+      block_sum_n<5>(f, sh.red_d2);
+      if (tid == 0) {
+        constexpr uint32_t KEY_ZERO = 0x80000000u, KEY_INF = 0xff800000u;
+        const bool t_inf = thr_key == KEY_INF, t_zero = thr_key == KEY_ZERO;
+        bool ok = true;
+        for (int j = 0; j < 4; ++j)
+          ok = ok && sh.ncand[rep[j]] <= CAND && sh.found[j] && sh.ext[j][0] <= sh.sel[j] && sh.sel[j] <= sh.ext[j][1];
+        ok = ok && (t_inf || t_zero || (sh.ext[1][0] < thr_key && thr_key < sh.ext[1][1]));
+        sh.lat_ok = ok;
+        if (ok) {
+          const long long fc_gt = (long long)f[2], fc_lt = (long long)f[3], fc_all = (long long)f[4];
+          double coarse_gt = 0, coarse_lt = 0;
+          long long cnt_gt = 0, sat[4] = {0, 0, 0, 0};
+          for (int q = 0; q < C; ++q) {
+            coarse_gt += sh.part_d[q][0]; coarse_lt += sh.part_d[q][1];
+            cnt_gt += sh.part_i[q][0];
+            for (int u = 0; u < 4; ++u) sat[u] += sh.part_i[q][1 + u];
+          }
+          const double thr = (double)key_float(thr_key);
+          const long long below = n - cnt_gt - sat[0] - sat[1] - fc_all;
+          const long long n_gt = cnt_gt + (t_inf ? 0 : sat[0]) + (t_zero ? 0 : sat[1]) + fc_gt;
+          const long long n_lt = below - (t_inf ? sat[2] : 0) - (t_zero ? sat[3] : 0) + fc_lt;
+          if (!t_inf && sat[0] > 0) coarse_gt += INFINITY;
+          const double sum_gt = fc_gt ? coarse_gt + f[0] : coarse_gt, sum_lt = fc_lt ? coarse_lt + f[1] : coarse_lt;
+          const long long n_eq = n - n_gt - n_lt;
+          const long long tt = K - n_gt;
+          sh.res_i[6] = tt;
+          sh.res_i[7] = n_eq - tt;
+          sh.res_d[1] = (sum_gt + (tt > 0 ? (double)tt * thr : 0.0)) / (double)K;
+          sh.res_d[2] = (sum_lt + (n_eq - tt > 0 ? (double)(n_eq - tt) * thr : 0.0)) / (double)(n - K);
+        }
+      }
+    }
+    cluster.sync();
+    STAMP();
+    radix = !L->lat_ok;
+#pragma unroll
+    for (int j = 0; j < 4; ++j) key_j[j] = L->sel[j];
+  }
+
+  if (radix) {
+    if (r == 0 && tid == 0) atomicAdd(reinterpret_cast<unsigned long long*>(header + TH_RADIX), 1ull);
+    for (int i = tid; i < SL1; i += SEL_THREADS) sh.hist[i] = 0;
+    cluster.sync();
+    STAMP();
+    {
+      a0 = 0;
+      c0 = 0;
+      sweep([&](float x, uint32_t c, bool in) {
+        a0 += (double)c * (double)x;
+        c0 += c;
+        warp_hist_add(sh.hist, float_key(x) >> 21, c, in);
+      });
+      STAMP();
+      push_hist(sh.hist, L->hist, SL1, r);
+      a0 = block_sum(a0, sh.red_d);
+      c0 = block_sum(c0, sh.red_i);
+      if (tid == 0) { L->part_d[r][0] = a0; L->part_i[r][0] = c0; }
+    }
+    cluster.sync();
+    STAMP();
+    if (r == 0) {
+      if (tid == 0) {
+        double sum_all = 0;
+        long long cnt_all = 0;
+        for (int q = 0; q < C; ++q) { sum_all += sh.part_d[q][0]; cnt_all += sh.part_i[q][0]; }
+        if (cnt_all != n) header[TH_MISMATCH] = 1;
+        const long long ninf = sh.hist[3], pinf = sh.hist[2044], nan = sh.hist[2047];
+        const long long hi_ = pinf + nan;
+        sh.res_i[0] = (hi_ + ninf) > 0; sh.res_i[1] = hi_ > 0 || ninf > n - K; sh.res_i[2] = hi_ > K || ninf > 0;
+        sh.res_i[3] = nan > 0; sh.res_i[4] = nan > 0; sh.res_i[5] = nan > K;
+        sh.res_d[0] = sum_all / (double)n;
+      }
+      scan_hists(sh.hist, SL1, 1, sh.warp_tot);
+      if (tid < 4) {
+        int bin; long long rem;
+        find_rank(sh.hist, SL1, ranks[tid], bin, rem);
+        sh.res_i[8 + tid] = bin; sh.res_i[12 + tid] = rem;
+      }
+    }
+    cluster.sync();
+    uint32_t pre[4];
+    long long rk[4];
+#pragma unroll
+    for (int j = 0; j < 4; ++j) { pre[j] = (uint32_t)L->res_i[8 + j]; rk[j] = L->res_i[12 + j]; }
+    STAMP();
+    int rep[4];
+    auto find_reps = [&]() {
+#pragma unroll
+      for (int j = 0; j < 4; ++j) {
+        rep[j] = j;
+#pragma unroll
+        for (int q = 3; q >= 0; --q)
+          if (q < j && pre[q] == pre[j]) rep[j] = q;
+      }
+    };
+    auto copy_reps = [&](int bins) {
+      for (int j = 1; j < 4; ++j)
+        if (rep[j] != j)
+          for (int i = tid; i < bins; i += SEL_THREADS) sh.hist[j * bins + i] = sh.hist[rep[j] * bins + i];
+      __syncthreads();
+    };
+    find_reps();
+
+    for (int j = 0; j < 4; ++j)
+      if (rep[j] == j)
+        for (int i = tid; i < SL2; i += SEL_THREADS) sh.hist[j * SL2 + i] = 0;
+    cluster.sync();
+    {
+      sweep([&](float x, uint32_t c, bool in) {
+        const uint32_t k = float_key(x);
+        const uint32_t b1 = k >> 21, b2 = (k >> 10) & (SL2 - 1);
+#pragma unroll
+        for (int j = 0; j < 4; ++j)
+          if (rep[j] == j) warp_hist_add(sh.hist + j * SL2, b2, c, in && b1 == pre[j]);
+      });
+      STAMP();
 #pragma unroll
       for (int j = 0; j < 4; ++j)
-        if (rep[j] == j) warp_hist_add(sh.hist + j * SL2, b2, c, in && b1 == pre[j]);
-    });
+        if (rep[j] == j) push_hist(sh.hist + j * SL2, L->hist + j * SL2, SL2, r);
+    }
     STAMP();
-#pragma unroll
+    cluster.sync();
+    STAMP();
+    if (r == 0) {
+      copy_reps(SL2);
+      scan_hists(sh.hist, SL2, 4, sh.warp_tot);
+      if (tid < 4) {
+        int bin; long long rem;
+        find_rank(sh.hist + tid * SL2, SL2, rk[tid], bin, rem);
+        sh.res_i[8 + tid] = bin; sh.res_i[12 + tid] = rem;
+      }
+    }
+    cluster.sync();
+#pragma unroll
+    for (int j = 0; j < 4; ++j) { pre[j] = (pre[j] << 11) | (uint32_t)L->res_i[8 + j]; rk[j] = L->res_i[12 + j]; }
+    find_reps();
+    STAMP();
+
     for (int j = 0; j < 4; ++j)
-      if (rep[j] == j) push_hist(sh.hist + j * SL2, L->hist + j * SL2, SL2, r);
-  }
-  STAMP();
-  cluster.sync();
-  STAMP();
-  if (r == 0) {
-    copy_reps(SL2);
-    scan_hists(sh.hist, SL2, 4, sh.warp_tot);
-    if (tid < 4) {
-      int bin; long long rem;
-      find_rank(sh.hist + tid * SL2, SL2, rk[tid], bin, rem);
-      sh.res_i[8 + tid] = bin; sh.res_i[12 + tid] = rem;
-    }
-  }
-  cluster.sync();
-#pragma unroll
-  for (int j = 0; j < 4; ++j) { pre[j] = (pre[j] << 11) | (uint32_t)L->res_i[8 + j]; rk[j] = L->res_i[12 + j]; }
-  find_reps();
-  STAMP();
-
-  for (int j = 0; j < 4; ++j)
-    if (rep[j] == j)
-      for (int i = tid; i < SL3; i += SEL_THREADS) sh.hist[j * SL3 + i] = 0;
-  cluster.sync();
-  const uint32_t thr22 = pre[1];
-  {
-    double v[2] = {0, 0};
-    long long c_gt = 0;
-    sweep([&](float x, uint32_t c, bool in) {
-      const uint32_t k = float_key(x);
-      const uint32_t hi22 = k >> 10;
-      const double cx = (double)c * (double)x;
-      if (in && hi22 > thr22) { v[0] += cx; c_gt += c; }
-      else if (in && hi22 < thr22) v[1] += cx;
+      if (rep[j] == j)
+        for (int i = tid; i < SL3; i += SEL_THREADS) sh.hist[j * SL3 + i] = 0;
+    cluster.sync();
+    const uint32_t thr22 = pre[1];
+    {
+      double v[2] = {0, 0};
+      long long c_gt = 0;
+      sweep([&](float x, uint32_t c, bool in) {
+        const uint32_t k = float_key(x);
+        const uint32_t hi22 = k >> 10;
+        const double cx = (double)c * (double)x;
+        if (in && hi22 > thr22) { v[0] += cx; c_gt += c; }
+        else if (in && hi22 < thr22) v[1] += cx;
+#pragma unroll
+        for (int j = 0; j < 4; ++j)
+          if (rep[j] == j) warp_hist_add(sh.hist + j * SL3, k & (SL3 - 1), c, in && hi22 == pre[j]);
+      });
+      STAMP();
 #pragma unroll
       for (int j = 0; j < 4; ++j)
-        if (rep[j] == j) warp_hist_add(sh.hist + j * SL3, k & (SL3 - 1), c, in && hi22 == pre[j]);
-    });
+        if (rep[j] == j) push_hist(sh.hist + j * SL3, L->hist + j * SL3, SL3, r);
+      STAMP();
+      block_sum_n<2>(v, sh.red_d2);
+      c_gt = block_sum(c_gt, sh.red_i);
+      if (tid == 0) { L->part_d[r][0] = v[0]; L->part_d[r][1] = v[1]; L->part_i[r][0] = c_gt; }
+    }
+    cluster.sync();
+    if (r == 0) {
+      copy_reps(SL3);
+      scan_hists(sh.hist, SL3, 4, sh.warp_tot);
+      if (tid < 4) {
+        int bin; long long rem;
+        find_rank(sh.hist + tid * SL3, SL3, rk[tid], bin, rem);
+        sh.res_i[8 + tid] = bin; sh.res_i[12 + tid] = rem;
+      }
+      __syncthreads();
+      const uint32_t thr_key = (pre[1] << 10) | (uint32_t)sh.res_i[8 + 1];
+      const uint32_t thr_lo = thr_key & (SL3 - 1), base = thr_key & ~(uint32_t)(SL3 - 1);
+      double f[5] = {0, 0, 0, 0, 0};
+      const uint32_t* h3 = sh.hist + 1 * SL3;
+      for (uint32_t b3 = tid; b3 < (uint32_t)SL3; b3 += SEL_THREADS) {
+        const long long c = (long long)h3[b3] - (b3 > 0 ? (long long)h3[b3 - 1] : 0);
+        f[4] += (double)c;
+        if (c == 0 || b3 == thr_lo) continue;
+        const double val = (double)c * (double)key_float(base | b3);
+        if (b3 > thr_lo) { f[0] += val; f[2] += (double)c; } else { f[1] += val; f[3] += (double)c; }
+      }
+      block_sum_n<5>(f, sh.red_d2);
+      if (tid == 0) {
+        const long long fc_gt = (long long)f[2], fc_lt = (long long)f[3], fc_all = (long long)f[4];
+        double coarse_gt = 0, coarse_lt = 0;
+        long long cnt_gt = 0;
+        for (int q = 0; q < C; ++q) { coarse_gt += sh.part_d[q][0]; coarse_lt += sh.part_d[q][1]; cnt_gt += sh.part_i[q][0]; }
+        const double thr = (double)key_float(thr_key);
+        const long long n_gt = cnt_gt + fc_gt, n_lt = (n - cnt_gt - fc_all) + fc_lt;
+        const double sum_gt = fc_gt ? coarse_gt + f[0] : coarse_gt, sum_lt = fc_lt ? coarse_lt + f[1] : coarse_lt;
+        const long long n_eq = n - n_gt - n_lt;
+        const long long tt = K - n_gt;
+        sh.res_i[6] = tt;
+        sh.res_i[7] = n_eq - tt;
+        sh.res_d[1] = (sum_gt + (tt > 0 ? (double)tt * thr : 0.0)) / (double)K;
+        sh.res_d[2] = (sum_lt + (n_eq - tt > 0 ? (double)(n_eq - tt) * thr : 0.0)) / (double)(n - K);
+      }
+    }
+    cluster.sync();
+#pragma unroll
+    for (int j = 0; j < 4; ++j) key_j[j] = (pre[j] << 10) | (uint32_t)L->res_i[8 + j];
     STAMP();
-#pragma unroll
-    for (int j = 0; j < 4; ++j)
-      if (rep[j] == j) push_hist(sh.hist + j * SL3, L->hist + j * SL3, SL3, r);
-    STAMP();
-    block_sum_n<2>(v, sh.red_d2);
-    c_gt = block_sum(c_gt, sh.red_i);
-    if (tid == 0) { L->part_d[r][0] = v[0]; L->part_d[r][1] = v[1]; L->part_i[r][0] = c_gt; }
-  }
-  cluster.sync();
-  if (r == 0) {
-    copy_reps(SL3);
-    scan_hists(sh.hist, SL3, 4, sh.warp_tot);
-    if (tid < 4) {
-      int bin; long long rem;
-      find_rank(sh.hist + tid * SL3, SL3, rk[tid], bin, rem);
-      sh.res_i[8 + tid] = bin; sh.res_i[12 + tid] = rem;
-    }
-    __syncthreads();
-    const uint32_t thr_key = (pre[1] << 10) | (uint32_t)sh.res_i[8 + 1];
-    const uint32_t thr_lo = thr_key & (SL3 - 1), base = thr_key & ~(uint32_t)(SL3 - 1);
-    double f[5] = {0, 0, 0, 0, 0};
-    const uint32_t* h3 = sh.hist + 1 * SL3;
-    for (uint32_t b3 = tid; b3 < (uint32_t)SL3; b3 += SEL_THREADS) {
-      const long long c = (long long)h3[b3] - (b3 > 0 ? (long long)h3[b3 - 1] : 0);
-      f[4] += (double)c;
-      if (c == 0 || b3 == thr_lo) continue;
-      const double val = (double)c * (double)key_float(base | b3);
-      if (b3 > thr_lo) { f[0] += val; f[2] += (double)c; } else { f[1] += val; f[3] += (double)c; }
-    }
-    block_sum_n<5>(f, sh.red_d2);
-    if (tid == 0) {
-      const long long fc_gt = (long long)f[2], fc_lt = (long long)f[3], fc_all = (long long)f[4];
-      double coarse_gt = 0, coarse_lt = 0;
-      long long cnt_gt = 0;
-      for (int q = 0; q < C; ++q) { coarse_gt += sh.part_d[q][0]; coarse_lt += sh.part_d[q][1]; cnt_gt += sh.part_i[q][0]; }
-      const double thr = (double)key_float(thr_key);
-      const long long n_gt = cnt_gt + fc_gt, n_lt = (n - cnt_gt - fc_all) + fc_lt;
-      const double sum_gt = fc_gt ? coarse_gt + f[0] : coarse_gt, sum_lt = fc_lt ? coarse_lt + f[1] : coarse_lt;
-      const long long n_eq = n - n_gt - n_lt;
-      const long long tt = K - n_gt;
-      sh.res_i[6] = tt;
-      sh.res_i[7] = n_eq - tt;
-      sh.res_d[1] = (sum_gt + (tt > 0 ? (double)tt * thr : 0.0)) / (double)K;
-      sh.res_d[2] = (sum_lt + (n_eq - tt > 0 ? (double)(n_eq - tt) * thr : 0.0)) / (double)(n - K);
-    }
-  }
-  cluster.sync();
-  uint32_t key_j[4];
-#pragma unroll
-  for (int j = 0; j < 4; ++j) key_j[j] = (pre[j] << 10) | (uint32_t)L->res_i[8 + j];
+  }
   const uint32_t thr_key = key_j[1];
-  const double mean_t = L->res_d[1], mean_j = L->res_d[2];
-  STAMP();
+  const double mean_a = L->res_d[0], mean_t = L->res_d[1], mean_j = L->res_d[2];
 
   double d[6] = {0, 0, 0, 0, 0, 0};
   sweep([&](float x, uint32_t ci, bool in) {
@@ -743,7 +1030,7 @@
 template <int K>
 static int launch_select_k(int n_grid, long long* header, const unsigned long long* ukeys, const uint32_t* ucnt,
                            float* wbuf, int64_t ldw, int32_t H, const LogTable& lf, double logV0, int64_t n_total,
-                           int64_t top, double* stats, bool beside_sweep, cudaStream_t st) {
+                           int64_t top, double* stats, bool beside_sweep, bool force_radix, cudaStream_t st) {
   static bool attr_set[64] = {false};
   int dev = 0;
   B200_CUDA(cudaGetDevice(&dev));
@@ -751,7 +1038,7 @@
   select_shape(C, cache);
   static const bool forced = getenv("B200_SELECT_CLUSTER") != nullptr;
   if (beside_sweep && !forced) C = 2;
-  const size_t dyn = (size_t)cache * 8;
+  const size_t dyn = (size_t)cache * 10;
   if (dev < 64 && !attr_set[dev]) {
     B200_CUDA(cudaFuncSetAttribute(tally_select_kernel<K>, cudaFuncAttributeMaxDynamicSharedMemorySize, (int)dyn));
     if (C > 8) B200_CUDA(cudaFuncSetAttribute(tally_select_kernel<K>, cudaFuncAttributeNonPortableClusterSizeAllowed, 1));
@@ -771,7 +1058,7 @@
   cfg.attrs = at;
   cfg.numAttrs = 1;
   return check_cuda(cudaLaunchKernelEx(&cfg, tally_select_kernel<K>, header, ukeys, ucnt, wbuf, ldw, H, lf, logV0,
-                                       n_total, top, stats, (int32_t)cache),
+                                       n_total, top, stats, (int32_t)cache, (int32_t)force_radix),
                     "tally_select launch");
 }
 
@@ -881,9 +1168,10 @@
     }
   const double logV0 = log((double)desc->value_0);
   const bool beside = (desc->flags & B200_LEV_FLAG_BESIDE_SWEEP) != 0;
+  const bool radix = (desc->flags & B200_LEV_FLAG_RADIX_SELECT) != 0;
   switch (desc->n_outcomes) {
-    case 2: return launch_select_k<2>(desc->n_grid, L.header, L.ukeys, L.ucnt, L.wbuf, L.ldw, desc->horizon, lf, logV0, n_total, top, stats, beside, st);
-    case 3: return launch_select_k<3>(desc->n_grid, L.header, L.ukeys, L.ucnt, L.wbuf, L.ldw, desc->horizon, lf, logV0, n_total, top, stats, beside, st);
-    default: return launch_select_k<4>(desc->n_grid, L.header, L.ukeys, L.ucnt, L.wbuf, L.ldw, desc->horizon, lf, logV0, n_total, top, stats, beside, st);
-  }
-}
+    case 2: return launch_select_k<2>(desc->n_grid, L.header, L.ukeys, L.ucnt, L.wbuf, L.ldw, desc->horizon, lf, logV0, n_total, top, stats, beside, radix, st);
+    case 3: return launch_select_k<3>(desc->n_grid, L.header, L.ukeys, L.ucnt, L.wbuf, L.ldw, desc->horizon, lf, logV0, n_total, top, stats, beside, radix, st);
+    default: return launch_select_k<4>(desc->n_grid, L.header, L.ukeys, L.ucnt, L.wbuf, L.ldw, desc->horizon, lf, logV0, n_total, top, stats, beside, radix, st);
+  }
+}
diff --git a/rlmd_b200/csrc/tally.cuh b/rlmd_b200/csrc/tally.cuh
--- a/rlmd_b200/csrc/tally.cuh
+++ b/rlmd_b200/csrc/tally.cuh
@@ -13,11 +13,14 @@
   TH_BAD = 2,
   TH_TIMEOUT = 3,
   TH_MISMATCH = 4,
+  TH_RADIX = 5,
   TH_TICKET = 9,
   TH_LISTPOS = 10,
   TH_CONCAT = 11,
   TH_DEBUG = 16,
-  TH_WORDS = 64
+  TH_BOX_ACC = 64,
+  TH_BOX = 68,
+  TH_WORDS = 72
 };
 
 struct TallyDev {
diff --git a/rlmd_b200/tally.py b/rlmd_b200/tally.py
--- a/rlmd_b200/tally.py
+++ b/rlmd_b200/tally.py
@@ -188,7 +188,7 @@
         self.rows = 0
 
     def stats(self, factors: np.ndarray, value_0: float, horizon: int, *, n_total: int, top: int,
-              beside_sweep: bool = False) -> torch.Tensor:
+              beside_sweep: bool = False, radix_select: bool = False) -> torch.Tensor:
         f = np.ascontiguousarray(factors, dtype=np.float32)
         if f.ndim != 2:
             raise ValueError("factors must be [G,K]")
@@ -197,7 +197,7 @@
         d = LevDesc()
         d.kind, d.mode, d.source = _lib.LEV_DISCRETE, _lib.MODE_LOG, _lib.SRC_STREAM
         d.horizon, d.n_outcomes, d.value_0 = int(horizon), k, float(value_0)
-        d.flags = _lib.LEV_FLAG_BESIDE_SWEEP if beside_sweep else 0
+        d.flags = (_lib.LEV_FLAG_BESIDE_SWEEP if beside_sweep else 0) | (_lib.LEV_FLAG_RADIX_SELECT if radix_select else 0)
         with torch.cuda.device(self.dev):
             for g0 in range(0, g, self.plan.grid_cap):
                 tile = np.ascontiguousarray(f[g0:g0 + self.plan.grid_cap])
@@ -216,7 +216,7 @@
             dist.all_reduce(w, op=dist.ReduceOp.MAX, group=self.group)
         w = w.cpu().tolist()
         return {"bins": w[0], "overflow": bool(w[1]), "bad_outcomes": w[2], "timed_out": bool(w[3]),
-                "count_mismatch": bool(w[4])}
+                "count_mismatch": bool(w[4]), "radix_route": w[5]}
 
     def check(self) -> dict:
         i = self.info()
```

Result: faster. 22080 billion, median of 6 (+3.1%).
